# tangjiapeng/NSDP

Hardware: AMD Instinct MI355X
Metric: query-points/sec fwd+bwd (2048 surf pts, 8192 queries) (higher is better)
Workload: dtype f32; 1 GPU; forward.yaml TDNet train step (fwd + l2 loss + bwd + Adam), 32 shapes/GPU, 2048 surface + 8192 query points per shape, fp32 (dense layers as bf16x3 split products), procedural random-init weights; global_batch=32, n_surf=2048, n_query=8192, parallelism=dp1

## Files before the change

include/nsdp_hip.h:

```cpp
#ifndef NSDP_HIP_H_
#define NSDP_HIP_H_

#include <stddef.h>
#include <stdint.h>

#ifdef __cplusplus
extern "C" {
#endif

#define NSDP_EINVAL (-1)
#define NSDP_ENOSUP (-2)

int nsdp_abi_version(void);
const char *nsdp_last_error(void);
void nsdp_debug_set(int key, int value);
int nsdp_device_count(void);


int nsdp_furthest_point_sampling(const float *xyz, int B, int N, int nsamples, float *tmp,
                                 int32_t *idx_out, void *stream);

int nsdp_gather_points(const float *points, const int32_t *idx, int B, int C, int N, int M,
                       float *out, void *stream);
int nsdp_gather_points_grad(const float *grad_out, const int32_t *idx, int B, int C, int N, int M,
                            float *grad_points, void *stream);

int nsdp_group_points(const float *points, const int32_t *idx, int B, int C, int N, int NP, int NS,
                      float *out, void *stream);
int nsdp_group_points_grad(const float *grad_out, const int32_t *idx, int B, int C, int N, int NP,
                           int NS, float *grad_points, void *stream);

int nsdp_scatter_cm_lists_supported(int B, int C, int N, int E);
int nsdp_scatter_cm_lists(const float *grad_out, const int32_t *offsets, const int32_t *entries, int B, int C, int N,
                          int E, float *grad_points, void *stream);

int nsdp_three_interpolate_grad_lists_supported(int B, int c, int n, int m);
int nsdp_three_interpolate_grad_lists(const float *grad_out, const float *weight, const int32_t *offsets,
                                      const int32_t *entries, int B, int c, int n, int m, float *grad_points, void *stream);


int nsdp_ball_query(const float *new_xyz, const float *xyz, int B, int N, int M, float radius,
                    int nsample, int32_t *idx_out, void *stream);

int nsdp_three_nn(const float *unknown, const float *known, int B, int n, int m, float *dist2,
                  int32_t *idx, void *stream);
int nsdp_three_interpolate(const float *points, const int32_t *idx, const float *weight, int B,
                           int c, int m, int n, float *out, void *stream);
int nsdp_three_interpolate_grad(const float *grad_out, const int32_t *idx, const float *weight,
                                int B, int c, int n, int m, float *grad_points, void *stream);


int nsdp_knn(const float *query, const float *source, int B, int n, int m, int k, int32_t *idx_out,
             float *dist2_out, void *stream);

int nsdp_knn_ragged(const float *query, const int32_t *offsets, const float *source, int B, int cap, int m, int k,
                    int32_t *idx_out, float *dist2_out, void *stream);

int nsdp_gather_rows(const float *points, const int32_t *idx, int B, int N, int C, int S, float *out,
                     void *stream);
int nsdp_rel_coords4(const float *query, const float *source, const int32_t *idx, int B, int n, int m, int k, float sign,
                     float *out4, void *stream);
int nsdp_scatter_add_rows(const float *grad_out, const int32_t *idx, int B, int N, int C, int S,
                          float *grad_points, void *stream);


int nsdp_linear_f32(const float *X, const float *W, const float *bias, const float *residual,
                    const float *mask, const float *out_mask, float *Y, long long M, int N, int K,
                    int relu_in, int relu_out, void *stream);

long long nsdp_packed_weight_floats(int N, int K);
int nsdp_pack_weight_f32(const float *W, int N, int K, float *Wp, float *WpT, void *stream);

int nsdp_linear_wp_f32(const float *X, const float *Wp, const float *bias, const float *residual,
                       const float *mask, const float *out_mask, float *Y, long long M, int N, int K,
                       int relu_in, int relu_out, void *stream);

typedef struct {
  const float *W;
  void *Wp;
  void *WpT;
  int N, K;
  int kind;
  int reserved;
} NsdpPackDesc;
int nsdp_pack_weights_batched(const NsdpPackDesc *descs, int count, void *stream);

typedef struct {
  float *param;
  const float *grad;
  float *exp_avg;
  float *exp_avg_sq;
  float *step;
  long long numel;
} NsdpAdamDesc;
int nsdp_adam_chunk_elems(void);
int nsdp_adam_multi_f32(const NsdpAdamDesc *descs_dev, const int32_t *chunks_dev, int n_chunks, int32_t *done_dev,
                        const float *lr_dev, double lr, double beta1, double beta2, double eps, double weight_decay,
                        int maximize, void *stream);

long long nsdp_packed_weight_bf16x3_bytes(int N, int K, int transposed);
int nsdp_pack_weight_bf16x3(const float *W, int N, int K, void *Wp, void *WpT, void *stream);
int nsdp_linear_bf16x3_f32(const float *X, const void *Wp, const float *bias, const float *residual,
                           const float *mask, const float *out_mask, float *Y, long long M, int N, int K,
                           int relu_in, int relu_out, void *stream);

int nsdp_linear_bf16x3_gather_f32(const float *X, const void *Wp, const float *bias, const float *gq, int g_div, const float *gk,
                                  const int32_t *gidx, int g_rows_per_shape, int g_nsrc, float *Y, long long M, int N, int K,
                                  int relu_in, int relu_out, void *stream);

int nsdp_linear_bf16x3_signed_f32(const float *X, const void *Wp, const float *bias, const float *residual, float residual_sign,
                                  float *Y, long long M, int N, int K, int relu_in, int relu_out, void *stream);

int nsdp_linear_bf16x3_addend_f32(const float *X, const void *Wp, const float *bias, const float *residual, const float *mask,
                                  const float *out_mask, const float *addend, float *Y, long long M, int N, int K,
                                  int relu_out, void *stream);

int nsdp_linear_bf16x3_h0_supported(long long M, int N, int K);
int nsdp_linear_bf16x3_h0_f32(const float *X4, const float *W0, const float *b0, const void *Wp, const float *bias,
                              const float *gq, int g_div, const float *gk, const int32_t *gidx, int g_rows_per_shape, int g_nsrc,
                              float *Y, long long M, int N, int K, void *stream);

int nsdp_linear_bf16x3_k4tail_ok(long long M, int N, int K);
size_t nsdp_linear_bf16x3_k4tail_workspace_bytes(long long M, int N);
int nsdp_linear_bf16x3_k4tail_f32(const float *dY, const void *WpT, const float *X4, const float *W0, const float *b0,
                                  float *dW0, float *db0, long long M, int N, int K, int k_out, int accumulate, float *ws,
                                  size_t ws_bytes, void *stream);


size_t nsdp_linear_wgrad_workspace_bytes(long long M, int N, int K);
int nsdp_linear_wgrad_f32(const float *dY, const float *X, const float *mask, int relu_x, float *dW,
                          float *db, long long M, int N, int K, int accumulate, float *workspace,
                          size_t workspace_bytes, void *stream);
int nsdp_linear_wgrad_k4_remask_f32(const float *dY, const float *X, const float *W, const float *bias, float *dW,
                                    float *db, long long M, int N, int accumulate, float *workspace,
                                    size_t workspace_bytes, void *stream);

int nsdp_linear_wgrad_bf16x3_supported(long long M, int N, int K);
size_t nsdp_linear_wgrad_bf16x3_workspace_bytes(long long M, int N, int K);
int nsdp_linear_wgrad_bf16x3_f32(const float *dY, const float *X, const float *mask, int relu_x, float *dW,
                                 float *db, long long M, int N, int K, int accumulate, float *workspace,
                                 size_t workspace_bytes, void *stream);

typedef struct {
  const float *ws;
  float *dW, *db;
  int S, nta, ktb;
  int N, K;
  int accumulate;
  int reserved;
} NsdpWgradReduceDesc;
int nsdp_linear_wgrad_bf16x3_partials_f32(const float *dY, const float *X, const float *mask, int relu_x, float *dW,
                                          float *db, long long M, int N, int K, int accumulate, float *workspace,
                                          size_t workspace_bytes, NsdpWgradReduceDesc *desc_out, void *stream);
int nsdp_wgrad_bf16x3_reduce_batched(const NsdpWgradReduceDesc *descs, int count, void *stream);

int nsdp_attn_pre_fwd_bf16(const void *q, const void *kf, const void *pos, const int32_t *idx, int B, int n, int N, int k,
                           int d, int q_per_shape, void *u, void *stream);
int nsdp_attn_pre_bwd_bf16(const void *du, const int32_t *idx, int B, int n, int N, int k, int d, int q_per_shape,
                           float *dq, float *dkf, void *dpos_acc, void *stream);
int nsdp_attn_post_fwd_bf16(const void *a, const void *vf, const void *pos, const int32_t *idx, const void *a_g,
                            const void *v_g, const void *residual, int B, int n, int N, int k, int d, void *y, float *lse,
                            void *stream);
int nsdp_attn_post_bwd_bf16(const void *dy, const void *a, const void *vf, const void *pos, const int32_t *idx,
                            const void *a_g, const void *v_g, const void *y, const void *residual, const float *lse, int B,
                            int n, int N, int k, int d, void *da, void *dpos, float *dvf, float *da_g, float *dv_g,
                            void *stream);

long long nsdp_packed_weight_bf16_bytes(int N, int K, int transposed);
int nsdp_pack_weights_bf16(const NsdpPackDesc *descs, int count, void *stream);
int nsdp_linear_bf16(const void *X, const void *Wp, const float *bias, const void *residual, const void *mask,
                     const void *out_mask, void *Y, long long M, int N, int K, int relu_in, int relu_out, int out_f32,
                     void *stream);
size_t nsdp_linear_wgrad_bf16_workspace_bytes(long long M, int N, int K);
int nsdp_linear_wgrad_bf16_takes_mask(long long M, int N, int K);
int nsdp_linear_wgrad_bf16(const void *dY, const void *X, const void *mask, int relu_x, float *dW, float *db,
                           long long M, int N, int K, int accumulate, float *workspace, size_t workspace_bytes,
                           void *stream);

int nsdp_linear_wgrad_bf16x3_h0_supported(long long M, int N, int K);
int nsdp_linear_wgrad_bf16x3_h0_f32(const float *dY, const float *X4, const float *W0, const float *b0, float *dW, float *db,
                                    long long M, int N, int K, int accumulate, float *workspace, size_t workspace_bytes,
                                    NsdpWgradReduceDesc *desc_out, void *stream);

int nsdp_layout_g16_f32(const float *src, float *dst, long long M, int C, int to_g16, void *stream);
int nsdp_linear_bf16x3_g16_supported(long long M, int N, int K, int layout, int has_mask, int relu_in);
int nsdp_linear_bf16x3_g16_f32(const float *X, const void *Wp, const float *bias, const float *residual, const float *mask,
                               const float *out_mask, const float *addend, float *Y, long long M, int N, int K, int relu_in,
                               int relu_out, int layout, const unsigned char *mask_bits, unsigned char *bits_out, void *stream);
size_t nsdp_relu_bits_bytes(long long M, int C);
int nsdp_linear_wgrad_bf16x3_g16_supported(long long M, int N, int K, int layout, int has_mask);
int nsdp_linear_wgrad_bf16x3_g16_f32(const float *dY, const float *X, const float *mask, int relu_x, float *dW, float *db,
                                     long long M, int N, int K, int accumulate, float *workspace, size_t workspace_bytes,
                                     NsdpWgradReduceDesc *desc_out, int layout, const unsigned char *mask_bits, void *stream);

typedef struct {
  const float *ws;
  float *dW, *db;
  int S, N, K;
  int accumulate;
  int reserved;
} NsdpWgradB16ReduceDesc;
int nsdp_linear_wgrad_bf16_partials(const void *dY, const void *X, const void *mask, int relu_x, float *dW, float *db,
                                    long long M, int N, int K, int accumulate, float *workspace, size_t workspace_bytes,
                                    NsdpWgradB16ReduceDesc *desc_out, void *stream);
int nsdp_wgrad_bf16_reduce_batched(const NsdpWgradB16ReduceDesc *descs, int count, void *stream);
int nsdp_linear_wgrad_partials_f32(const float *dY, const float *X, const float *mask, int relu_x, float *dW, float *db,
                                   long long M, int N, int K, int accumulate, float *workspace, size_t workspace_bytes,
                                   NsdpWgradB16ReduceDesc *desc_out, void *stream);

int nsdp_bn_stats_bf16(const void *x, const void *addend, long long R, int C, float eps, float momentum,
                       float *running_mean, float *running_var, float *mean, float *invstd, float *workspace,
                       long long *num_batches_tracked, void *stream);
int nsdp_bn_train_fwd_bf16(const void *x, const void *addend, long long R, int C, float eps, float momentum, int updates,
                           float *running_mean, float *running_var, long long *num_batches_tracked, const float *gamma,
                           const float *beta, int relu, void *y, float *mean, float *invstd, float *workspace,
                           void *stream);
int nsdp_bn_apply_bf16(const void *x, const void *addend, const float *mean, const float *invstd, const float *gamma,
                       const float *beta, long long R, int C, int relu, void *y, void *stream);
int nsdp_bn_backward_bf16(const void *dy, const void *y_relu, const void *x, const void *addend, const float *mean,
                          const float *invstd, const float *gamma, long long R, int C, int training, void *dx,
                          float *dgamma, float *dbeta, float *workspace, void *stream);

int nsdp_knn_invert(const int32_t *idx, int B, int E, int N, int32_t *offsets, int32_t *entries, void *stream);
int nsdp_segment_sum_rows(const float *src, const int32_t *offsets, const int32_t *entries, int B, int E, int N, int d,
                          float scale, float *out, void *stream);
int nsdp_segment_sum_rows_bf16(const void *src, const int32_t *offsets, const int32_t *entries, int B, int E, int N, int d,
                               float scale, float *out, void *stream);
int nsdp_segment_sum_rows_add(const float *src, const int32_t *offsets, const int32_t *entries, int B, int E, int N, int d,
                              float scale, const float *addend, float *out, void *stream);
int nsdp_segment_sum_rows_add_bf16(const void *src, const int32_t *offsets, const int32_t *entries, int B, int E, int N, int d,
                                   float scale, const float *addend, float *out, void *stream);

size_t nsdp_scatter_rows_onehot_bf16_workspace_bytes(int B, long long rows, int N, int d);
int nsdp_scatter_rows_onehot_bf16(const void *src, const int32_t *idx, int B, long long rows, int N, int d, float *table,
                                  float *workspace, size_t workspace_bytes, void *stream);
size_t nsdp_scatter_rows_onehot_f32_workspace_bytes(int B, long long rows, int N, int d);
int nsdp_scatter_rows_onehot_f32(const float *src, const int32_t *idx, int B, long long rows, int N, int d, float *table,
                                 float *workspace, size_t workspace_bytes, void *stream);

int nsdp_linear_k4_bf16(const float *X, const float *W, const float *bias, void *Y, long long M, int N, int relu_out,
                        void *stream);
size_t nsdp_linear_wgrad_k4_bf16_workspace_bytes(long long M, int N);
int nsdp_linear_wgrad_k4_bf16(const void *dY, const float *X, const void *mask, float *dW, float *db, long long M, int N,
                              float *workspace, size_t workspace_bytes, void *stream);


int nsdp_attn_pre_fwd(const float *q, const float *kf, const float *pos, const int32_t *idx, int B, int n,
                      int N, int k, int d, int q_per_shape, float *u, void *stream);
int nsdp_attn_pre_bwd(const float *du, const int32_t *idx, int B, int n, int N, int k, int d,
                      int q_per_shape, float *dq, float *dkf, float *dpos_acc, void *stream);
int nsdp_attn_pre_bwd_sub(const float *du, const int32_t *idx, int B, int n, int N, int k, int d, const float *dq_sub, float *dq,
                          void *stream);
int nsdp_attn_pre_bwd_sub_bf16(const void *du, const int32_t *idx, int B, int n, int N, int k, int d, const void *dq_sub, float *dq,
                               void *stream);
int nsdp_attn_post_fwd(const float *a, const float *vf, const float *pos, const int32_t *idx,
                       const float *a_g, const float *v_g, const float *residual, int B, int n, int N,
                       int k, int d, float *y, float *lse, void *stream);
int nsdp_attn_post_bwd(const float *dy, const float *a, const float *vf, const float *pos,
                       const int32_t *idx, const float *a_g, const float *v_g, const float *y,
                       const float *residual, const float *lse, int B, int n, int N, int k, int d,
                       float *da, float *dpos, float *dvf, float *da_g, float *dv_g, void *stream);

int nsdp_attn_post_fwd_q(const float *a, const float *vk, const float *u, const int32_t *idx, const float *qsub,
                         const float *residual, int B, int n, int N, int k, int d, float *y, float *lse, void *stream);
int nsdp_attn_post_bwd_q(const float *dy, const float *a, const float *vk, const float *u, const int32_t *idx, const float *qsub,
                         const float *y, const float *residual, const float *lse, int B, int n, int N, int k, int d,
                         float *da, float *dpos, float *dvf, void *stream);

size_t nsdp_attn_post_bwd_det_workspace_bytes(int B, int n, int k, int d);
int nsdp_attn_post_bwd_det(const float *dy, const float *a, const float *vf, const float *pos, const int32_t *idx,
                           const float *a_g, const float *v_g, const float *y, const float *residual, const float *lse,
                           int B, int n, int N, int k, int d, float *da, float *dpos, float *da_g, float *dv_g,
                           float *workspace, size_t workspace_bytes, void *stream);
int nsdp_attn_post_bwd_det_bf16(const void *dy, const void *a, const void *vf, const void *pos, const int32_t *idx,
                                const void *a_g, const void *v_g, const void *y, const void *residual, const float *lse,
                                int B, int n, int N, int k, int d, void *da, void *dpos, float *da_g, float *dv_g,
                                float *workspace, size_t workspace_bytes, void *stream);


int nsdp_decoder_fused_fwd(const float *xyz_q, const float *anchors, const int32_t *idx, const float *qk,
                           const float *vtab, const float *a_g, const float *v_g,
                           const float *const *weights, int n_weights, int B, int NQ, int A, int KN, int D,
                           int H, float *out, void *stream);

int nsdp_decoder_fused_fwd_bf16(const float *xyz_q, const float *anchors, const int32_t *idx, const float *qk,
                                const float *vtab, const float *a_g, const float *v_g,
                                const void *const *weights, int n_weights, int B, int NQ, int A, int KN, int D,
                                int H, float *out, void *stream);

int nsdp_decoder_fused_fwd_ragged(const float *xyz_q, const int32_t *offsets, const float *anchors, const int32_t *idx,
                                  const float *qk, const float *vtab, const float *a_g, const float *v_g,
                                  const float *const *weights, int n_weights, int B, int cap, int A, int KN, int D,
                                  int H, float *out, void *stream);
int nsdp_decoder_fused_fwd_bf16_ragged(const float *xyz_q, const int32_t *offsets, const float *anchors, const int32_t *idx,
                                       const float *qk, const float *vtab, const float *a_g, const float *v_g,
                                       const void *const *weights, int n_weights, int B, int cap, int A, int KN, int D,
                                       int H, float *out, void *stream);

size_t nsdp_bn_workspace_bytes(int C);
int nsdp_bn_stats(const float *x, const float *addend, long long R, int C, float eps, float momentum,
                  float *running_mean, float *running_var, float *mean, float *invstd, float *workspace,
                  long long *num_batches_tracked, void *stream);
int nsdp_bn_train_fwd(const float *x, const float *addend, long long R, int C, float eps, float momentum, int updates,
                      float *running_mean, float *running_var, long long *num_batches_tracked, const float *gamma,
                      const float *beta, int relu, float *y, float *mean, float *invstd, float *workspace, void *stream);
int nsdp_bn_apply(const float *x, const float *addend, const float *mean, const float *invstd,
                  const float *gamma, const float *beta, long long R, int C, int relu, float *y, void *stream);
int nsdp_bn_backward(const float *dy, const float *y_relu, const float *x, const float *addend,
                     const float *mean, const float *invstd, const float *gamma, long long R, int C,
                     int training, float *dx, float *dgamma, float *dbeta, float *workspace, void *stream);

void nsdp_prof_enable(int on);
void nsdp_prof_enable_kinds(unsigned mask);
int nsdp_prof_num_kinds(void);
void nsdp_trace_enable(int on);
int nsdp_trace_read(char *buf, int capacity);
const char *nsdp_prof_name(int kind);
int nsdp_prof_collect(int kind, long long *launches, double *total_ms, double *flops, double *bytes);

int nsdp_graph_exec_create(void *graph, int max_streams, void **out_handle);
int nsdp_graph_exec_info(void *handle, int *nodes, int *kernels, int *streams, int *cross_edges, int *own_graph_nodes);
int nsdp_graph_exec_launch(void *handle, void *stream);
int nsdp_graph_exec_launch_timed(void *handle, void *stream, const char *name_substr, long long *launches, double *total_ms);
int nsdp_graph_exec_destroy(void *handle);

#ifdef __cplusplus
}
#endif
#endif
```

nsdp_amd/build.py:

```python
from __future__ import annotations

import os
import subprocess
import sys
from concurrent.futures import ThreadPoolExecutor

HERE = os.path.dirname(os.path.abspath(__file__))
CSRC = os.path.join(HERE, "csrc")
LIBDIR = os.path.join(HERE, "lib")
OBJDIR = os.path.join(LIBDIR, "obj")
SO = os.path.join(LIBDIR, "libnsdp_hip.so")
HEADER = os.path.join(os.path.dirname(HERE), "include", "nsdp_hip.h")

HIPCC = os.environ.get("HIPCC", "/opt/rocm/bin/hipcc")
COMMON = ["--offload-arch=gfx950", "-O3", "-std=c++17", "-fPIC", "-Wall", "-Wno-unused-function",
          "-munsafe-fp-atomics"]
EXACT = ["-ffp-contract=off"]
FAST = ["-ffp-contract=fast"]
PER_FILE = {
    "fps.hip": EXACT,
    "knn.hip": EXACT,
    "pointnet2_ops.hip": EXACT,
    "adam.hip": EXACT,
    "wgrad_bf16x3.hip": FAST + ["-O2", "-fno-slp-vectorize"],
    "gemm_bf16x3.hip": FAST + ["-fno-slp-vectorize"],
    "gemm_bf16x3_g16.hip": FAST + ["-fno-slp-vectorize"],
}


def sources():
    return sorted(f for f in os.listdir(CSRC) if f.endswith(".hip"))


def _deps_mtime():
    hs = [os.path.join(CSRC, f) for f in os.listdir(CSRC) if f.endswith(".h")] + [HEADER, os.path.abspath(__file__)]
    return max(os.path.getmtime(h) for h in hs)


def _compile(src, force):
    obj = os.path.join(OBJDIR, src[:-4] + ".o")
    path = os.path.join(CSRC, src)
    if (not force and os.path.exists(obj)
            and os.path.getmtime(obj) >= max(os.path.getmtime(path), _deps_mtime())):
        return obj, False
    cmd = [HIPCC] + COMMON + PER_FILE.get(src, FAST) + ["-c", path, "-o", obj]
    subprocess.check_call(cmd)
    return obj, True


def build(force: bool = False, verbose: bool = False) -> str:
    os.makedirs(OBJDIR, exist_ok=True)
    with ThreadPoolExecutor(max_workers=min(8, os.cpu_count() or 1)) as ex:
        results = list(ex.map(lambda s: _compile(s, force), sources()))
    objs = [o for o, _ in results]
    if force or any(c for _, c in results) or not os.path.exists(SO):
        subprocess.check_call([HIPCC, "--offload-arch=gfx950", "-shared", "-fPIC", "-o", SO] + objs)
        if verbose:
            print("linked", SO)
    return SO


if __name__ == "__main__":
    print(build(force="--force" in sys.argv, verbose=True))
```

nsdp_amd/csrc/x3_kernel.h:

```cpp
#pragma once
#include <stdlib.h>

#include <type_traits>

#include "common.h"
#include "k4.h"
#include "pack_bodies.h"
#include "prof.h"

namespace nsdp {
extern int g_x3_dbg;
extern thread_local int g_x3_side_reserve;
}

namespace {

using f32x4 = __attribute__((ext_vector_type(4))) float;
using f32x2 = __attribute__((ext_vector_type(2))) float;
using u32x4 = __attribute__((ext_vector_type(4))) unsigned;
using bf16x2 = __attribute__((ext_vector_type(2))) __bf16;
using bf16x8 = __attribute__((ext_vector_type(8))) __bf16;

typedef __attribute__((address_space(3))) void *lds_ptr_t;
typedef const __attribute__((address_space(1))) void *gbl_ptr_t;

using nsdp::g_x3_dbg;
using nsdp::g_x3_side_reserve;

#ifdef NSDP_X3_TIMING
__device__ unsigned long long g_x3_timers[8];
#define X3_T(var) const unsigned long long var = __builtin_readcyclecounter()
#define X3_ADD(i, a, b) t_acc[i] += (b) - (a)
#else
#define X3_T(var)
#define X3_ADD(i, a, b)
#endif

struct X3Params {
  const float *X;
  const void *Wp;
  const float *bias, *residual, *mask, *out_mask;
  float *Y;
  long long M;
  int N, K;
  int relu_in, relu_out;
  int dbg;
  const float *gq, *gk;
  const int32_t *gidx;
  int g_div, g_rps, g_nsrc;
  float res_sign = 1.f;
  const float *addend = nullptr;
  const float *t_x4 = nullptr, *t_w0 = nullptr, *t_b0 = nullptr;
  float *t_ws = nullptr;
  const float *h_x4 = nullptr, *h_w0 = nullptr, *h_b0 = nullptr;
  const unsigned char *bits = nullptr;
  unsigned char *bits_out = nullptr;
};

constexpr int kLayX = 1;
constexpr int kLayY = 2;
constexpr int kLayR = 4;

__device__ __forceinline__ void split_pair(float x0, float x1, unsigned &h, unsigned &m, unsigned &l) {
  h = __builtin_bit_cast(unsigned, __builtin_convertvector(f32x2{x0, x1}, bf16x2));
  const float r0 = x0 - __builtin_bit_cast(float, h << 16), r1 = x1 - __builtin_bit_cast(float, h & 0xffff0000u);
  m = __builtin_bit_cast(unsigned, __builtin_convertvector(f32x2{r0, r1}, bf16x2));
  const float s0 = r0 - __builtin_bit_cast(float, m << 16), s1 = r1 - __builtin_bit_cast(float, m & 0xffff0000u);
  l = __builtin_bit_cast(unsigned, __builtin_convertvector(f32x2{s0, s1}, bf16x2));
}

__device__ __forceinline__ f32x4 mfma_bf16(u32x4 a, u32x4 b, f32x4 c) {
  return __builtin_amdgcn_mfma_f32_16x16x32_bf16(__builtin_bit_cast(bf16x8, a), __builtin_bit_cast(bf16x8, b), c, 0, 0, 0);
}

template <int I, int N, typename F>
__device__ __forceinline__ void static_for(F &&f) {
  if constexpr (I < N) {
    f(std::integral_constant<int, I>{});
    static_for<I + 1, N>(f);
  }
}

#define NSDP_DPP4(CTRL, A, B, C, D)                                                                                              \
  asm("s_nop 1\n\t"                                                                                                              \
      "v_add_f32_dpp %0, %0, %0 " CTRL "\n\tv_add_f32_dpp %1, %1, %1 " CTRL "\n\tv_add_f32_dpp %2, %2, %2 " CTRL "\n\t"            \
      "v_add_f32_dpp %3, %3, %3 " CTRL "\n\ts_nop 1"                                                                              \
      : "+v"(A), "+v"(B), "+v"(C), "+v"(D))
#define NSDP_DPP16(CTRL, T)                                                                                                      \
  asm("s_nop 1\n\t"                                                                                                              \
      "v_add_f32_dpp %0, %0, %0 " CTRL "\n\tv_add_f32_dpp %1, %1, %1 " CTRL "\n\tv_add_f32_dpp %2, %2, %2 " CTRL "\n\t"            \
      "v_add_f32_dpp %3, %3, %3 " CTRL "\n\tv_add_f32_dpp %4, %4, %4 " CTRL "\n\tv_add_f32_dpp %5, %5, %5 " CTRL "\n\t"            \
      "v_add_f32_dpp %6, %6, %6 " CTRL "\n\tv_add_f32_dpp %7, %7, %7 " CTRL "\n\tv_add_f32_dpp %8, %8, %8 " CTRL "\n\t"            \
      "v_add_f32_dpp %9, %9, %9 " CTRL "\n\tv_add_f32_dpp %10, %10, %10 " CTRL "\n\tv_add_f32_dpp %11, %11, %11 " CTRL "\n\t"      \
      "v_add_f32_dpp %12, %12, %12 " CTRL "\n\tv_add_f32_dpp %13, %13, %13 " CTRL "\n\tv_add_f32_dpp %14, %14, %14 " CTRL "\n\t"   \
      "v_add_f32_dpp %15, %15, %15 " CTRL "\n\ts_nop 1"                                                                           \
      : "+v"(T[0]), "+v"(T[1]), "+v"(T[2]), "+v"(T[3]), "+v"(T[4]), "+v"(T[5]), "+v"(T[6]), "+v"(T[7]), "+v"(T[8]), "+v"(T[9]),   \
        "+v"(T[10]), "+v"(T[11]), "+v"(T[12]), "+v"(T[13]), "+v"(T[14]), "+v"(T[15]))
template <bool K3>
__device__ __forceinline__ void row16_sum20(float (&t)[20]) {
  if constexpr (K3) {
    float u[16] = {t[0], t[1], t[2], t[4], t[5], t[6], t[8], t[9], t[10], t[12], t[13], t[14], t[16], t[17], t[18], t[19]};
    NSDP_DPP16("quad_perm:[1,0,3,2] row_mask:0xf bank_mask:0xf", u);
    NSDP_DPP16("quad_perm:[2,3,0,1] row_mask:0xf bank_mask:0xf", u);
    NSDP_DPP16("row_half_mirror row_mask:0xf bank_mask:0xf", u);
    NSDP_DPP16("row_mirror row_mask:0xf bank_mask:0xf", u);
    t[0] = u[0]; t[1] = u[1]; t[2] = u[2]; t[4] = u[3]; t[5] = u[4]; t[6] = u[5]; t[8] = u[6]; t[9] = u[7]; t[10] = u[8];
    t[12] = u[9]; t[13] = u[10]; t[14] = u[11]; t[16] = u[12]; t[17] = u[13]; t[18] = u[14]; t[19] = u[15];
  } else {
    NSDP_DPP16("quad_perm:[1,0,3,2] row_mask:0xf bank_mask:0xf", t);
    NSDP_DPP4("quad_perm:[1,0,3,2] row_mask:0xf bank_mask:0xf", t[16], t[17], t[18], t[19]);
    NSDP_DPP16("quad_perm:[2,3,0,1] row_mask:0xf bank_mask:0xf", t);
    NSDP_DPP4("quad_perm:[2,3,0,1] row_mask:0xf bank_mask:0xf", t[16], t[17], t[18], t[19]);
    NSDP_DPP16("row_half_mirror row_mask:0xf bank_mask:0xf", t);
    NSDP_DPP4("row_half_mirror row_mask:0xf bank_mask:0xf", t[16], t[17], t[18], t[19]);
    NSDP_DPP16("row_mirror row_mask:0xf bank_mask:0xf", t);
    NSDP_DPP4("row_mirror row_mask:0xf bank_mask:0xf", t[16], t[17], t[18], t[19]);
  }
}
#undef NSDP_DPP16
#undef NSDP_DPP4

__device__ __forceinline__ void xload(f32x4 &dst, const float *lane_ptr) {
  asm volatile("global_load_dwordx4 %0, %1, off" : "=v"(dst) : "v"(lane_ptr));
}
__device__ __forceinline__ void bload(unsigned &dst, const unsigned char *lane_ptr) {
  asm volatile("global_load_ubyte %0, %1, off" : "=v"(dst) : "v"(lane_ptr));
}


template <int OFF>
__device__ __forceinline__ void lds_read(u32x4 &dst, unsigned lane_addr) {
  asm volatile("ds_read_b128 %0, %1 offset:%2" : "=v"(dst) : "v"(lane_addr), "n"(OFF));
}
__device__ __forceinline__ void lds_wait(u32x4 &a, u32x4 &b, u32x4 &c) {
  asm volatile("s_waitcnt lgkmcnt(0)" : "+v"(a), "+v"(b), "+v"(c));
}

typedef __attribute__((address_space(3))) f32x4 *lds_f4_ptr;
template <int OFF>
__device__ __forceinline__ void lds_read_f4(f32x4 &dst, unsigned addr) {
  dst = *reinterpret_cast<lds_f4_ptr>(static_cast<uintptr_t>(addr + static_cast<unsigned>(OFF)));
}
template <int OFF>
__device__ __forceinline__ void lds_write_f4(unsigned addr, f32x4 v) {
  *reinterpret_cast<lds_f4_ptr>(static_cast<uintptr_t>(addr + static_cast<unsigned>(OFF))) = v;
}
template <int CNT>
__device__ __forceinline__ void lgkm_wait(f32x4 &) {}
__device__ __forceinline__ void store_f4(unsigned byte_off, f32x4 v, float *uniform_base) {
  *reinterpret_cast<f32x4 *>(reinterpret_cast<char *>(uniform_base) + byte_off) = v;
}

template <int MT, int NT, int PRE, int WV, bool XREG = false, int KBM = 2, int GATHER = 0, int TAIL = 0, int LAY = 0>
__global__ __launch_bounds__(WV * 64, XREG ? 2 : 1) void linear_bf16x3_kernel(X3Params p) {
  constexpr bool kXG = (LAY & kLayX) != 0, kYG = (LAY & kLayY) != 0, kRG = (LAY & kLayR) != 0;
  static_assert(!kYG || (!GATHER && !TAIL), "G16 output: plain epilogue forms");
  static_assert(!kXG || PRE != 3, "G16 input: there is no X in the H0 forms");
  static_assert(PRE != 4 || kXG, "ReLU bits belong to G16 operands");
  constexpr bool kMasked = PRE == 1 || PRE == 4;
  static_assert(!GATHER || PRE == 0 || PRE == 3, "the gathered addend belongs to the plain-prologue forms");
  static_assert(!TAIL || (PRE == 0 && !GATHER), "the K = 4 tail belongs to the plain-prologue forms");
  constexpr bool WRES = KBM > 2;
  constexpr bool kH0 = PRE == 3;
  constexpr bool kXLds = !kMasked && !XREG && !kH0;
  constexpr int kWTile = NT * 3 * 64;
  constexpr int kXTile = kXLds ? 2 * WV * MT * 2 * 64 : 1;
  constexpr bool kTwoPerCu = XREG || (NT <= 8 && WV == 4);
  constexpr int kCap = (kTwoPerCu ? 80 : 160) * 64;
  constexpr int kBiasLds = NT * 4;
  constexpr int kH0Rows = kH0 ? ((NT * 16 + 31) / 32) * 32 : 0;
  constexpr int kH0XRows = kH0 ? 2 * WV * MT * 16 : 0;
  constexpr int kH0Lds = kH0Rows + kH0Rows / 4 + kH0XRows;
  constexpr int kExtFree = kCap - KBM * kWTile - kXTile - kBiasLds - kH0Lds;
  constexpr bool kStage = !WRES && kExtFree >= 0 && !TAIL && !kYG;
  constexpr int kExtWant = WV * NT * 64 - kWTile;
  constexpr int kExt = !kStage ? 0 : (kExtWant < 0 ? 0 : (kExtFree < 0 ? 0 : (kExtWant < kExtFree ? kExtWant : kExtFree)));
  constexpr int kPerWave = (kWTile + kExt) / WV;
  constexpr int kTppFit = kPerWave / 64 < NT ? kPerWave / 64 : NT;
  constexpr int kTppCap = (NT == 13 && (WV == 8 || XREG)) ? 5 : 8;
  constexpr int kTppMax = kTppFit < kTppCap ? kTppFit : kTppCap;
  constexpr int kPasses = kStage ? (NT + kTppMax - 1) / kTppMax : 1;
  constexpr int kTpp = (NT + kPasses - 1) / kPasses;
  static_assert(!kStage || kTppMax >= 1, "epilogue staging: no room for a 16 x 16 tile per wave");
  __shared__ __attribute__((aligned(16))) u32x4 wlds[KBM * kWTile + kExt];
  __shared__ __attribute__((aligned(16))) u32x4 xbuf[kXLds ? 2 : 1][kXLds ? WV : 1][kXLds ? MT * 2 * 64 : 1];
  __shared__ __attribute__((aligned(16))) float bias_lds[(kStage || TAIL) ? NT * 16 : 4];
  __shared__ __attribute__((aligned(16))) f32x4 t_w0lds[TAIL ? NT * 16 : 1];
  __shared__ __attribute__((aligned(16))) f32x4 t_x4lds[TAIL ? WV * 64 : 1];
  __shared__ __attribute__((aligned(16))) f32x4 h_w0lds[kH0 ? kH0Rows : 1];
  __shared__ __attribute__((aligned(16))) float h_b0lds[kH0 ? kH0Rows : 4];
  __shared__ __attribute__((aligned(16))) f32x4 h_x4lds[kH0 ? 2 : 1][kH0 ? WV : 1][kH0 ? MT * 16 : 1];
  static_assert(!TAIL || !WRES, "the K = 4 tail needs 1 KiB of LDS per wave and 272 B per n tile next to the weight buffers");
  static_assert(!TAIL || MT * 16 <= 64, "the K = 4 tail stages one input row per lane");
  auto wbuf_at = [&](int b) -> u32x4 * { return wlds + b * kWTile + (b >= 1 ? kExt : 0); };
  const int lane = threadIdx.x & 63;
  const int wave = __builtin_amdgcn_readfirstlane(threadIdx.x >> 6);
  const int li = lane & 15, g = lane >> 4;
  const int K = p.K, N = p.N;
  const int KB = (K + 31) >> 5;
  const int ntiles = (N + 15) >> 4;
  constexpr long long kRowsWg = static_cast<long long>(WV) * MT * 16;
  const long long wg_tiles = (p.M + kRowsWg - 1) / kRowsWg;
  const long long stride = gridDim.x;
  long long tile = blockIdx.x;

  const float *xa[MT], *xn[MT];
  const float *ma[MT], *mn[MT];
  auto set_rows = [&](long long t, const float **x, const float **m) {
#pragma unroll
    for (int mt = 0; mt < MT; ++mt) {
      long long r = (t * WV + wave) * (MT * 16) + mt * 16 + li;
      r = r < p.M ? r : (p.M - 1);
      const long long ro = kXG ? (r & ~15LL) * K + (r & 15) * 4 : r * K;
      x[mt] = p.X + ro;
      m[mt] = PRE == 1 ? p.mask + ro : nullptr;
      if constexpr (PRE == 4)
        m[mt] = reinterpret_cast<const float *>(p.bits + (r >> 4) * (static_cast<long long>((K + 31) >> 5) * 64) + (r & 15) * 4 + g);
    }
  };
  set_rows(tile, xa, ma);
  set_rows(tile + stride, xn, mn);
  f32x4 h_xs[kH0 ? MT : 1];
  int h_kb = 0;
  unsigned h_par = 0;
  auto h_rows = [&](long long t, unsigned buf) {
    if (lane < MT * 16) {
      long long r = (t * WV + wave) * (MT * 16) + lane;
      r = r < p.M ? r : (p.M - 1);
      __builtin_amdgcn_global_load_lds((gbl_ptr_t)(p.h_x4 + r * 4), (lds_ptr_t)(&h_x4lds[buf][wave][0]), 16, 0, 0);
    }
  };
  auto h_take = [&](unsigned buf) {
#pragma unroll
    for (int mt = 0; mt < MT; ++mt) h_xs[mt] = h_x4lds[buf][wave][mt * 16 + li];
  };
  if constexpr (kH0) {
    h_rows(tile, 0u);
    h_rows(tile + stride, 1u);
    asm volatile("s_waitcnt vmcnt(0)" ::: "memory");
    h_take(0u);
  }

  const char *wlane = static_cast<const char *>(p.Wp) + lane * 16;
  auto stage = [&](int kb, int buf) {
    const int pieces = ntiles * 3;
    for (int q = wave; q < pieces; q += WV)
      __builtin_amdgcn_global_load_lds((gbl_ptr_t)(wlane + ((static_cast<long long>(kb) * pieces + q) << 10)),
                                       (lds_ptr_t)(wbuf_at(buf) + q * 64), 16, 0, 0);
  };
  const unsigned lds0 = static_cast<unsigned>(reinterpret_cast<uintptr_t>((lds_ptr_t)(&wlds[lane])));
  const unsigned ldsw = static_cast<unsigned>(reinterpret_cast<uintptr_t>((lds_ptr_t)(&wlds[0])));
  const unsigned ldsb = static_cast<unsigned>(reinterpret_cast<uintptr_t>((lds_ptr_t)(&bias_lds[0])));
  constexpr unsigned kBufBytes = NT * 3 * 1024;
  constexpr unsigned kExtBytes = kExt * 16;

  f32x4 raw[kXLds ? 1 : MT][2], rawm[kXLds ? 1 : MT][2];
  unsigned rawb[PRE == 4 ? MT : 1];
  auto xissue = [&](const float *const *x, const float *const *m, int kb, unsigned xb) {
    if constexpr (kH0) return;
#pragma unroll
    for (int mt = 0; mt < MT; ++mt)
#pragma unroll
      for (int hf = 0; hf < 2; ++hf) {
        int ko = kb * 32 + 16 * hf + 4 * g;
        ko = ko < K ? ko : (K - 4);
        if constexpr (kXG) ko *= 16;
        if constexpr (kXLds) {
          const float *src = x[mt] + ko;
          if (p.dbg & 1024) src = x[0] - li * K + (((kb * MT * 2 + mt * 2 + hf) * 256) % 6144) + lane * 4;
          __builtin_amdgcn_global_load_lds((gbl_ptr_t)src, (lds_ptr_t)(&xbuf[xb][wave][(mt * 2 + hf) * 64]), 16, 0, 0);
        } else {
          xload(raw[mt][hf], x[mt] + ko);
          if constexpr (PRE == 1) xload(rawm[mt][hf], m[mt] + ko);
          if constexpr (PRE == 4) {
            if (hf == 0) bload(rawb[mt], reinterpret_cast<const unsigned char *>(m[mt]) + kb * 64);
          }
        }
      }
  };
  auto xwait = [&]() {
    if constexpr (kXLds || kH0) {
      asm volatile("s_waitcnt vmcnt(0)" ::: "memory");
    } else {
#pragma unroll
      for (int mt = 0; mt < MT; ++mt) {
        asm volatile("s_waitcnt vmcnt(0)" : "+v"(raw[mt][0]), "+v"(raw[mt][1]));
        if constexpr (PRE == 1) asm volatile("s_waitcnt vmcnt(0)" : "+v"(rawm[mt][0]), "+v"(rawm[mt][1]));
        if constexpr (PRE == 4) asm volatile("s_waitcnt vmcnt(0)" : "+v"(rawb[mt]));
      }
    }
  };
  struct Planes {
    u32x4 h[MT], m[MT], l[MT];
  };
  auto convert_pair = [&](Planes &pl, int mt, int pr, unsigned xb) {
    if constexpr (kH0) {
      const int k0 = h_kb * 32 + 16 * (pr >> 1) + 4 * g + 2 * (pr & 1);
      const f32x4 wa = h_w0lds[k0], wb = h_w0lds[k0 + 1];
      const f32x2 bb = *reinterpret_cast<const f32x2 *>(&h_b0lds[k0]);
      const float4 xq = make_float4(h_xs[mt][0], h_xs[mt][1], h_xs[mt][2], h_xs[mt][3]);
      const f32x2 pre = nsdp::k4_preact_pair(xq, f32x2{wa[0], wa[1]}, f32x2{wa[2], wa[3]}, f32x2{wb[0], wb[1]}, f32x2{wb[2], wb[3]}, bb);
      unsigned h, m, l;
      split_pair(fmaxf(pre[0], 0.f), fmaxf(pre[1], 0.f), h, m, l);
      pl.h[mt][pr] = h; pl.m[mt][pr] = m; pl.l[mt][pr] = l;
      return;
    }
    f32x4 v;
    if constexpr (kXLds) {
      v = __builtin_bit_cast(f32x4, xbuf[xb][wave][(mt * 2 + (pr >> 1)) * 64 + lane]);
    } else {
      v = raw[mt][pr >> 1];
      if constexpr (PRE == 1) {
        const f32x4 mk = rawm[mt][pr >> 1];
#pragma unroll
        for (int c = 0; c < 4; ++c) v[c] = mk[c] > 0.f ? v[c] : 0.f;
      }
      if constexpr (PRE == 4) {
        const unsigned nib = rawb[mt] >> (4 * (pr >> 1));
#pragma unroll
        for (int c = 0; c < 4; ++c) v[c] = ((nib >> c) & 1u) ? v[c] : 0.f;
      }
    }
    if (PRE == 2) {
#pragma unroll
      for (int c = 0; c < 4; ++c) v[c] = __builtin_amdgcn_fmed3f(v[c], 0.f, __builtin_inff());
    }
    unsigned h, m, l;
    split_pair(v[2 * (pr & 1)], v[2 * (pr & 1) + 1], h, m, l);
    pl.h[mt][pr] = h; pl.m[mt][pr] = m; pl.l[mt][pr] = l;
  };

  auto pair_mt = [](int i) { return kH0 ? i % MT : i >> 2; };
  auto pair_pr = [](int i) { return kH0 ? i / MT : i & 3; };
  Planes cur, nxt;
  if constexpr (kH0) {
    for (int c = threadIdx.x; c < kH0Rows; c += WV * 64) h_b0lds[c] = (p.h_b0 && c < K) ? p.h_b0[c] : 0.f;
    for (int j = threadIdx.x; j < kH0Rows / 2; j += WV * 64) nsdp::k4_pair_table(p.h_w0, K, j, h_w0lds[2 * j], h_w0lds[2 * j + 1]);
    __syncthreads();
  }
  if constexpr (kStage) {
    for (int c = threadIdx.x; c < NT * 16; c += WV * 64) bias_lds[c] = (p.bias && c < p.N) ? p.bias[c] : 0.f;
  }
  if constexpr (TAIL) {
    for (int c = threadIdx.x; c < NT * 16; c += WV * 64) {
      bias_lds[c] = (p.t_b0 && c < p.N) ? p.t_b0[c] : 0.f;
      t_w0lds[c] = c < p.N ? *reinterpret_cast<const f32x4 *>(p.t_w0 + static_cast<long long>(c) * 4) : f32x4{0.f, 0.f, 0.f, 0.f};
    }
  }
  if (wg_tiles >= 4 * stride) {
    int phase = static_cast<int>(blockIdx.x & 7);
    if (WV == 4 && gridDim.x > 256 && blockIdx.x >= gridDim.x / 2) phase = (phase + 4) & 7;
    for (int i = 0; i < phase * KB; ++i) __builtin_amdgcn_s_sleep(10);
  }
  if constexpr (WRES) {
    for (int kb = 0; kb < KB; ++kb) stage(kb, kb);
  } else {
    stage(0, 0);
  }
  xissue(xa, ma, 0, 0u);
  if constexpr (kXLds) xissue(xa, ma, 1, 1u);
  xwait();
#pragma unroll
  for (int mt = 0; mt < MT; ++mt)
#pragma unroll
    for (int pr = 0; pr < 4; ++pr) convert_pair(cur, mt, pr, 0u);
  if constexpr (!kXLds) {
    xissue(xa, ma, 1, 0u);
    xwait();
  }
  __syncthreads();

  constexpr int kConvSteps = NT > 4 ? 4 : NT - 1;
  constexpr int kConvFirst = kXLds ? NT - kConvSteps : 0;
  constexpr int kPairs = MT * 4;
  constexpr int kPerStep = (kPairs + kConvSteps - 1) / kConvSteps;
  constexpr int kValuPerMfma = (kPerStep * ((PRE == 1 || PRE == 4) ? 13 : PRE == 2 ? 10 : PRE == 3 ? 21 : 9) + 6 * MT - 1) / (6 * MT);

#ifdef NSDP_X3_TIMING
  unsigned long long t_acc[8] = {0, 0, 0, 0, 0, 0, 0, 0};
  const unsigned long long t_begin = __builtin_readcyclecounter();
#endif
  unsigned gs = 0;
  for (;;) {
    X3_T(t_tile0);
    const long long row0 = (tile * WV + wave) * (MT * 16);
    const bool next_tile = tile + stride < wg_tiles;
    if constexpr (TAIL) {
      long long r = row0 + (lane < MT * 16 ? lane : MT * 16 - 1);
      r = r < p.M ? r : p.M - 1;
      __builtin_amdgcn_global_load_lds((gbl_ptr_t)(p.t_x4 + r * 4), (lds_ptr_t)(&t_x4lds[wave * 64]), 16, 0, 0);
    }
    int li_t = li, g_t = g;
    asm volatile("" : "+v"(li_t), "+v"(g_t));
    f32x4 acc[MT][NT];
    unsigned gqo[GATHER == 1 ? MT : 1], gko[GATHER ? MT : 1];
    if constexpr (GATHER) {
#pragma unroll
      for (int mt = 0; mt < MT; ++mt) {
        long long row = row0 + mt * 16 + li_t;
        row = row < p.M ? row : (p.M - 1);
        const unsigned r32 = static_cast<unsigned>(row);
        if constexpr (GATHER == 1) gqo[mt] = (r32 / static_cast<unsigned>(p.g_div)) * static_cast<unsigned>(N);
        gko[mt] = ((r32 / static_cast<unsigned>(p.g_rps)) * static_cast<unsigned>(p.g_nsrc) + static_cast<unsigned>(p.gidx[row])) *
                  static_cast<unsigned>(N);
      }
    }
    if (!GATHER && p.residual) {
#pragma unroll
      for (int mt = 0; mt < MT; ++mt) {
        long long row = row0 + mt * 16 + li_t;
        row = row < p.M ? row : (p.M - 1);
#pragma unroll
        for (int nt = 0; nt < NT; ++nt) {
          int col = nt * 16 + 4 * g_t;
          col = col + 4 <= N ? col : (N - 4);
          const long long ro = kRG ? (row & ~15LL) * N + (row & 15) * 4 + col * 16 : row * N + col;
          const float4 v = *reinterpret_cast<const float4 *>(p.residual + ro);
          acc[mt][nt] = f32x4{v.x, v.y, v.z, v.w};
          if constexpr (PRE == 0) acc[mt][nt] *= p.res_sign;
        }
      }
    } else {
#pragma unroll
      for (int mt = 0; mt < MT; ++mt)
#pragma unroll
        for (int nt = 0; nt < NT; ++nt) acc[mt][nt] = f32x4{0.f, 0.f, 0.f, 0.f};
    }

    X3_T(t_tile1);
    X3_ADD(4, t_tile0, t_tile1);
    for (int kb = 0; kb < KB; ++kb, ++gs) {
      X3_T(t_k0);
      const unsigned buf = gs & 1u;
      const bool more = kb + 1 < KB || next_tile;
      if constexpr (!WRES) {
        if (more && !(p.dbg & 1)) stage(kb + 1 < KB ? kb + 1 : 0, buf ^ 1u);
      }
      bool x_issued = false;
      if constexpr (kXLds) {
        if (kb + 2 < KB) { xissue(xa, ma, kb + 2, buf); x_issued = true; }
        else if (next_tile) { xissue(xn, mn, kb + 2 - KB, buf); x_issued = true; }
      }
      auto xwait_older = [&]() {
        if (x_issued) asm volatile("s_waitcnt vmcnt(%0)" ::"n"(MT * 2) : "memory");
        else asm volatile("s_waitcnt vmcnt(0)" ::: "memory");
      };
      if constexpr (kH0) {
        const bool wrap = kb + 1 >= KB;
        h_kb = wrap ? 0 : kb + 1;
        if (wrap) h_take(h_par ^ 1u);
      }
      const unsigned wsel = WRES ? static_cast<unsigned>(kb) : buf;
      const unsigned wl_addr = lds0 + wsel * kBufBytes + (wsel >= 1u ? kExtBytes : 0u);
      u32x4 wh, wm, wl;
      lds_read<0>(wh, wl_addr); lds_read<1024>(wm, wl_addr); lds_read<2048>(wl, wl_addr);
      lds_wait(wh, wm, wl);
      static_for<0, NT>([&](auto I) {
        constexpr int nt = decltype(I)::value;
        u32x4 nh, nm, nl;
        if constexpr (nt + 1 < NT) {
          lds_read<(nt + 1) * 3072>(nh, wl_addr);
          if (!(p.dbg & 512)) {
            lds_read<(nt + 1) * 3072 + 1024>(nm, wl_addr);
            lds_read<(nt + 1) * 3072 + 2048>(nl, wl_addr);
          } else {
            nm = nh; nl = nh;
          }
        }
        if constexpr (!kXLds && !kH0 && nt == kConvFirst + kConvSteps) {
          if (kb + 2 < KB) xissue(xa, ma, kb + 2, 0u);
          else if (next_tile) xissue(xn, mn, kb + 2 - KB, 0u);
        }
        if constexpr (kXLds && nt == kConvFirst) xwait_older();
        if constexpr (nt >= kConvFirst && nt < kConvFirst + kConvSteps) {
#pragma unroll
          for (int i = 0; i < kPerStep; ++i) {
            constexpr int base = (nt - kConvFirst) * kPerStep;
            if (base + i < kPairs) convert_pair(nxt, pair_mt(base + i), pair_pr(base + i), buf ^ 1u);
          }
        }
#pragma unroll
        for (int mt = 0; mt < MT; ++mt) acc[mt][nt] = mfma_bf16(wh, cur.l[mt], acc[mt][nt]);
#pragma unroll
        for (int mt = 0; mt < MT; ++mt) acc[mt][nt] = mfma_bf16(wl, cur.h[mt], acc[mt][nt]);
#pragma unroll
        for (int mt = 0; mt < MT; ++mt) acc[mt][nt] = mfma_bf16(wm, cur.m[mt], acc[mt][nt]);
#pragma unroll
        for (int mt = 0; mt < MT; ++mt) acc[mt][nt] = mfma_bf16(wh, cur.m[mt], acc[mt][nt]);
#pragma unroll
        for (int mt = 0; mt < MT; ++mt) acc[mt][nt] = mfma_bf16(wm, cur.h[mt], acc[mt][nt]);
#pragma unroll
        for (int mt = 0; mt < MT; ++mt) acc[mt][nt] = mfma_bf16(wh, cur.h[mt], acc[mt][nt]);
        if constexpr (nt >= kConvFirst && nt < kConvFirst + kConvSteps) {
#pragma unroll
          for (int i = 0; i < 6 * MT; ++i) {
            __builtin_amdgcn_sched_group_barrier(0x008, 1, 0);
            __builtin_amdgcn_sched_group_barrier(0x002, kValuPerMfma, 0);
          }
        }
#pragma unroll
        for (int mt = 0; mt < MT; ++mt) asm volatile("" : "+a"(acc[mt][nt]));
        if constexpr (nt >= kConvFirst && nt < kConvFirst + kConvSteps) {
#pragma unroll
          for (int i = 0; i < kPerStep; ++i) {
            constexpr int base = (nt - kConvFirst) * kPerStep;
            if (base + i < kPairs) {
              const int mt = pair_mt(base + i), pr = pair_pr(base + i);
              asm volatile("" : "+v"(nxt.h[mt][pr]), "+v"(nxt.m[mt][pr]), "+v"(nxt.l[mt][pr]));
            }
          }
        }
        if constexpr (nt + 1 < NT) {
          lds_wait(nh, nm, nl);
          wh = nh; wm = nm; wl = nl;
        }
      });
      X3_T(t_k1);
      if constexpr (kXLds) xwait_older();
      else xwait();
      X3_T(t_k2);
      if constexpr (!WRES) {
        asm volatile("s_waitcnt lgkmcnt(0)" ::: "memory");
        __builtin_amdgcn_s_barrier();
      }
      asm volatile("" ::: "memory");
      X3_T(t_k3);
      X3_ADD(0, t_k0, t_k1); X3_ADD(1, t_k1, t_k2); X3_ADD(2, t_k2, t_k3);
      cur = nxt;
    }

    X3_T(t_e0);
    if (row0 < p.M && !(p.dbg & 8)) {
      const bool full_rows = row0 + MT * 16 <= p.M;
      int li_e = li, g_e = g;
      asm volatile("" : "+v"(li_e), "+v"(g_e));
      float4 bias4[NT];
#pragma unroll
      for (int nt = 0; nt < NT; ++nt) bias4[nt] = make_float4(0.f, 0.f, 0.f, 0.f);
      if (p.bias && (!kStage || (p.dbg & (8192 | 16384 | 32768)))) {
#pragma unroll
        for (int nt = 0; nt < NT; ++nt) {
          const int col = nt * 16 + 4 * g_e;
          bias4[nt] = *reinterpret_cast<const float4 *>(p.bias + (col + 4 <= N ? col : (N - 4)));
        }
      }
      auto gload = [&](int nt, f32x4 *ga, f32x4 *gb) {
        if constexpr (GATHER) {
          int col = nt * 16 + 4 * g_e;
          col = col + 4 <= N ? col : (N - 4);
#pragma unroll
          for (int mt = 0; mt < MT; ++mt) {
            if constexpr (GATHER == 1) ga[mt] = *reinterpret_cast<const f32x4 *>(p.gq + gqo[mt] + col);
            gb[mt] = *reinterpret_cast<const f32x4 *>(p.gk + gko[mt] + col);
          }
        }
      };
      auto otile = [&](int nt, auto has_omask, auto guarded, const f32x4 *ga = nullptr, const f32x4 *gb = nullptr) {
        const int col = nt * 16 + 4 * g_e;
        const bool cv = col + 4 <= N;
        const int colc = cv ? col : (N - 4);
        const float4 bv = bias4[nt];
#pragma unroll
        for (int mt = 0; mt < MT; ++mt) {
          const long long row = row0 + mt * 16 + li_e;
          const bool rv = !decltype(guarded)::value || row < p.M;
          const long long rowc = rv ? row : (p.M - 1);
          float4 v = make_float4(acc[mt][nt][0] + bv.x, acc[mt][nt][1] + bv.y, acc[mt][nt][2] + bv.z, acc[mt][nt][3] + bv.w);
          if constexpr (GATHER) {
            const f32x4 d = GATHER == 2 ? gb[mt] : ga[mt] - gb[mt];
            v.x += d[0]; v.y += d[1]; v.z += d[2]; v.w += d[3];
          }
          if (p.relu_out) { v.x = fmaxf(v.x, 0.f); v.y = fmaxf(v.y, 0.f); v.z = fmaxf(v.z, 0.f); v.w = fmaxf(v.w, 0.f); }
          if (decltype(has_omask)::value) {
            const float4 om = *reinterpret_cast<const float4 *>(p.out_mask + rowc * N + colc);
            v.x = om.x > 0.f ? v.x : 0.f; v.y = om.y > 0.f ? v.y : 0.f; v.z = om.z > 0.f ? v.z : 0.f; v.w = om.w > 0.f ? v.w : 0.f;
          }
          if constexpr (decltype(has_omask)::value == 2) {
            const float4 ad = *reinterpret_cast<const float4 *>(p.addend + rowc * N + colc);
            v.x += ad.x; v.y += ad.y; v.z += ad.z; v.w += ad.w;
          }
          const f32x4 vv = {v.x, v.y, v.z, v.w};
          if (decltype(guarded)::value) {
            if (cv && rv) {
              if (p.dbg & 64) __builtin_nontemporal_store(vv, reinterpret_cast<f32x4 *>(p.Y + rowc * N + colc));
              else *reinterpret_cast<f32x4 *>(p.Y + rowc * N + colc) = vv;
            }
          } else {
            if (p.dbg & 64) __builtin_nontemporal_store(vv, reinterpret_cast<f32x4 *>(p.Y + row * N + col));
            else if (p.dbg & 2048)
              *reinterpret_cast<f32x4 *>(p.Y + row0 * N + (((mt * NT + nt) * 256) % 6144) + (li_e + 16 * g_e) * 4) = vv;
            else *reinterpret_cast<f32x4 *>(p.Y + row * N + col) = vv;
          }
        }
      };
      auto staged = [&](auto has_omask) {
        const unsigned buf_last = (gs - 1u) & 1u;
        const unsigned ebase = ldsw + (buf_last ? kBufBytes : 0u) + static_cast<unsigned>(wave) * (kPerWave * 16u);
        const unsigned lane_e = static_cast<unsigned>(li_e + 16 * g_e);
        const unsigned rd = ebase + lane_e * 16u;
        float *ytile = p.Y + row0 * N;
        const float *mtile = decltype(has_omask)::value ? p.out_mask + row0 * N : nullptr;
        const float *atile = decltype(has_omask)::value == 2 ? p.addend + row0 * N : nullptr;
        const int rows_left = p.M - row0 < MT * 16 ? static_cast<int>(p.M - row0) : MT * 16;
        static_for<0, MT>([&](auto MI) {
          constexpr int mt = decltype(MI)::value;
          static_for<0, kPasses>([&](auto PI) {
            constexpr int pass = decltype(PI)::value;
            constexpr int nt0 = pass * kTpp;
            constexpr int ntn = (NT - nt0) < kTpp ? (NT - nt0) : kTpp;
            constexpr unsigned pitch = ntn * 64u;
            const unsigned wr = ebase + static_cast<unsigned>(li_e) * pitch + static_cast<unsigned>(g_e) * 16u;
            const int valid = (N - nt0 * 16) * 4 < static_cast<int>(pitch) ? (N - nt0 * 16) * 4 : static_cast<int>(pitch);
            unsigned off[ntn];
            bool live[ntn];
            f32x4 om[decltype(has_omask)::value ? ntn : 1];
            f32x4 ad[decltype(has_omask)::value == 2 ? ntn : 1];
            f32x4 gka[GATHER == 2 ? ntn : 1];
            static_for<0, ntn>([&](auto CI) {
              constexpr int i = decltype(CI)::value;
              const unsigned f = static_cast<unsigned>(i) * 1024u + lane_e * 16u;
              const unsigned r = f / pitch, cb = f - r * pitch;
              off[i] = ((static_cast<unsigned>(mt) * 16u + r) * static_cast<unsigned>(N) + static_cast<unsigned>(nt0) * 16u) * 4u + cb;
              live[i] = static_cast<int>(cb) < valid && static_cast<int>(mt * 16 + r) < rows_left;
              if constexpr (decltype(has_omask)::value) {
                om[i] = live[i] ? *reinterpret_cast<const f32x4 *>(reinterpret_cast<const char *>(mtile) + off[i]) : f32x4{0.f, 0.f, 0.f, 0.f};
              }
              if constexpr (decltype(has_omask)::value == 2) {
                ad[i] = live[i] ? *reinterpret_cast<const f32x4 *>(reinterpret_cast<const char *>(atile) + off[i]) : f32x4{0.f, 0.f, 0.f, 0.f};
              }
              if constexpr (GATHER == 2) {
                const unsigned cbytes = static_cast<unsigned>(nt0) * 64u + cb;
                const unsigned ko = static_cast<unsigned>(__builtin_amdgcn_ds_bpermute(static_cast<int>(r * 4u), static_cast<int>(gko[mt])));
                gka[i] = live[i] ? *reinterpret_cast<const f32x4 *>(reinterpret_cast<const char *>(p.gk + ko) + cbytes) : f32x4{0.f, 0.f, 0.f, 0.f};
              }
            });
            f32x4 gav[GATHER == 1 ? ntn : 1], gbv[GATHER == 1 ? ntn : 1];
            if constexpr (GATHER == 1) {
              static_for<0, ntn>([&](auto TI) {
                constexpr int t = decltype(TI)::value;
                int col = (nt0 + t) * 16 + 4 * g_e;
                col = col + 4 <= N ? col : (N - 4);
                gav[t] = *reinterpret_cast<const f32x4 *>(p.gq + gqo[mt] + col);
                gbv[t] = *reinterpret_cast<const f32x4 *>(p.gk + gko[mt] + col);
              });
            }
            f32x4 bvv[ntn];
            static_for<0, ntn>([&](auto TI) {
              constexpr int t = decltype(TI)::value;
              lds_read_f4<(nt0 + t) * 64>(bvv[t], ldsb + static_cast<unsigned>(16 * g_e));
            });
            static_for<0, ntn>([&](auto TI) {
              constexpr int t = decltype(TI)::value;
              constexpr int nt = nt0 + t;
              lgkm_wait<ntn - 1 - t>(bvv[t]);
              f32x4 v = acc[mt][nt] + bvv[t];
              if constexpr (GATHER == 1) v += gav[t] - gbv[t];
              if (p.relu_out) {
#pragma unroll
                for (int c = 0; c < 4; ++c) v[c] = fmaxf(v[c], 0.f);
              }
              lds_write_f4<t * 64>(wr, v);
            });
            asm volatile("s_waitcnt lgkmcnt(0)" ::: "memory");
            f32x4 back[ntn];
            static_for<0, ntn>([&](auto CI) {
              constexpr int i = decltype(CI)::value;
              lds_read_f4<i * 1024>(back[i], rd);
            });
            static_for<0, ntn>([&](auto CI) {
              constexpr int i = decltype(CI)::value;
              lgkm_wait<ntn - 1 - i>(back[i]);
              f32x4 v = back[i];
              if constexpr (decltype(has_omask)::value) {
#pragma unroll
                for (int c = 0; c < 4; ++c) v[c] = om[i][c] > 0.f ? v[c] : 0.f;
              }
              if constexpr (decltype(has_omask)::value == 2) v += ad[i];
              if constexpr (GATHER == 2) v += gka[i];
              if (live[i]) store_f4(off[i], v, ytile);
            });
          });
        });
      };
      auto direct_tail = [&]() __attribute__((always_inline)) {
        f32x4 xr[MT];
        bool rvm[MT];
        const unsigned x4a = static_cast<unsigned>(reinterpret_cast<uintptr_t>((lds_ptr_t)(&t_x4lds[wave * 64]))) + static_cast<unsigned>(li_e) * 16u;
        const unsigned w0a = static_cast<unsigned>(reinterpret_cast<uintptr_t>((lds_ptr_t)(&t_w0lds[0]))) + static_cast<unsigned>(g_e) * 64u;
        static_for<0, MT>([&](auto MI) {
          constexpr int mt = decltype(MI)::value;
          rvm[mt] = row0 + mt * 16 + li_e < p.M;
          lds_read_f4<mt * 256>(xr[mt], x4a);
        });
        float *wsp = p.t_ws + (tile * WV + wave) * static_cast<long long>(NT * 80) + g_e * 20;
        static_for<0, NT>([&](auto NI) {
          constexpr int nt = decltype(NI)::value;
          const int col = nt * 16 + 4 * g_e;
          const bool cv = col < N;
          f32x4 w0[4], b0;
          static_for<0, 4>([&](auto CI) {
            constexpr int c = decltype(CI)::value;
            lds_read_f4<(nt * 16 + c) * 16>(w0[c], w0a);
          });
          lds_read_f4<nt * 64>(b0, ldsb + static_cast<unsigned>(16 * g_e));
          float ta[20];
#pragma unroll
          for (int v = 0; v < 20; ++v) ta[v] = 0.f;
#pragma unroll
          for (int mt = 0; mt < MT; ++mt) {
            const float4 xq = make_float4(xr[mt][0], xr[mt][1], xr[mt][2], xr[mt][3]);
            const bool ok = rvm[mt] && cv;
#pragma unroll
            for (int c = 0; c < 4; ++c) {
              const float pre = nsdp::k4_preact_n(xq, make_float4(w0[c][0], w0[c][1], w0[c][2], w0[c][3]), b0[c], c);
              const float d = (ok && pre > 0.f) ? acc[mt][nt][c] : 0.f;
              ta[16 + c] += d;
#pragma unroll
              for (int k = 0; k < (TAIL == 2 ? 3 : 4); ++k) ta[4 * c + k] += d * xr[mt][k];
            }
          }
          row16_sum20<TAIL == 2>(ta);
          if (li_e == 0) {
#pragma unroll
            for (int j = 0; j < 5; ++j)
              *reinterpret_cast<f32x4 *>(wsp + nt * 80 + j * 4) = f32x4{ta[4 * j], ta[4 * j + 1], ta[4 * j + 2], ta[4 * j + 3]};
          }
        });
      };
      auto g16_out = [&]() __attribute__((always_inline)) {
        float *ytile = p.Y + row0 * N + (li_e + 16 * g_e) * 4;
        unsigned char *btile = p.bits_out ? p.bits_out + (row0 >> 4) * (static_cast<long long>((N + 31) >> 5) * 64) + li_e * 4 + g_e : nullptr;
        static_for<0, MT>([&](auto MI) __attribute__((always_inline)) {
          constexpr int mt = decltype(MI)::value;
          if (row0 + mt * 16 < p.M) {
            unsigned byte = 0;
            static_for<0, NT>([&](auto NI) __attribute__((always_inline)) {
              constexpr int nt = decltype(NI)::value;
              const float4 bv = bias4[nt];
              f32x4 v = {acc[mt][nt][0] + bv.x, acc[mt][nt][1] + bv.y, acc[mt][nt][2] + bv.z, acc[mt][nt][3] + bv.w};
              if (p.relu_out) {
#pragma unroll
                for (int c = 0; c < 4; ++c) v[c] = fmaxf(v[c], 0.f);
              }
              const bool cv = nt * 16 + 4 * g_e + 4 <= N;
              if (cv) *reinterpret_cast<f32x4 *>(ytile + mt * 16 * N + nt * 256) = v;
              if (btile) {
                const unsigned nib = cv ? ((v[0] > 0.f ? 1u : 0u) | (v[1] > 0.f ? 2u : 0u) | (v[2] > 0.f ? 4u : 0u) | (v[3] > 0.f ? 8u : 0u)) : 0u;
                byte = (nt & 1) ? (byte | (nib << 4)) : nib;
                if ((nt & 1) || nt == NT - 1) {
                  if (nt * 16 < ((N + 31) >> 5) * 32) btile[mt * (((N + 31) >> 5) * 64) + (nt >> 1) * 64] = static_cast<unsigned char>(byte);
                }
              }
            });
          }
        });
      };
      auto epilogue = [&](auto has_omask) {
        const int full_tiles = N >> 4;
        if constexpr (TAIL) {
          direct_tail();
          return;
        }
        if constexpr (kYG) {
          g16_out();
          return;
        }
        if constexpr (kStage) {
          staged(has_omask);
          return;
        }
        if constexpr (GATHER) {
          f32x4 ga[2][MT], gb[2][MT];
          gload(0, ga[0], gb[0]);
          static_for<0, NT>([&](auto I) {
            constexpr int nt = decltype(I)::value;
            if (nt * 16 < N) {
              if constexpr (nt + 1 < NT) {
                if ((nt + 1) * 16 < N) gload(nt + 1, ga[(nt + 1) & 1], gb[(nt + 1) & 1]);
              }
              otile(nt, has_omask, std::true_type{}, ga[nt & 1], gb[nt & 1]);
            }
          });
          return;
        }
        if (full_rows) {
#pragma unroll
          for (int nt = 0; nt < NT; ++nt) {
            if (nt < full_tiles) otile(nt, has_omask, std::false_type{});
            else if (nt * 16 < N) otile(nt, has_omask, std::true_type{});
          }
        } else {
#pragma unroll
          for (int nt = 0; nt < NT; ++nt)
            if (nt * 16 < N) otile(nt, has_omask, std::true_type{});
        }
      };
      if (p.out_mask) {
        if constexpr (kMasked) {
          if (p.addend) epilogue(std::integral_constant<int, 2>{});
          else epilogue(std::true_type{});
        } else {
          epilogue(std::true_type{});
        }
      } else {
        epilogue(std::false_type{});
      }
    }

    X3_T(t_e1);
    X3_ADD(3, t_e0, t_e1);
    if (!next_tile) break;
    if constexpr (kStage) {
      asm volatile("s_waitcnt lgkmcnt(0)" ::: "memory");
      __builtin_amdgcn_s_barrier();
      asm volatile("" ::: "memory");
    }
    tile += stride;
#pragma unroll
    for (int mt = 0; mt < MT; ++mt) { xa[mt] = xn[mt]; ma[mt] = mn[mt]; }
    set_rows(tile + stride, xn, mn);
    if constexpr (kH0) {
      h_rows(tile + stride, h_par);
      h_par ^= 1u;
    }
  }
#ifdef NSDP_X3_TIMING
  t_acc[5] = __builtin_readcyclecounter() - t_begin;
  if (lane == 0)
    for (int i = 0; i < 6; ++i) atomicAdd(&g_x3_timers[i], t_acc[i]);
#endif
}

template <int MT, int NT, int PRE, int WV, bool XREG = false, int KBM = 2, int GATHER = 0, int LAY = 0>
void launch_x3_pre(const X3Params &p, hipStream_t st, int wgs_per_cu = 1) {
  const long long rows_per_wg = static_cast<long long>(WV) * MT * 16;
  const long long wg_tiles = (p.M + rows_per_wg - 1) / rows_per_wg;
  static const int reserve_env = getenv("NSDP_X3_RESERVE_CUS") ? atoi(getenv("NSDP_X3_RESERVE_CUS")) : 0;
  const int reserve = g_x3_side_reserve > 0 && g_x3_side_reserve < nsdp::num_cus() ? g_x3_side_reserve : reserve_env;
  const long long slots = static_cast<long long>(nsdp::num_cus() - reserve) * wgs_per_cu;
  const unsigned grid = static_cast<unsigned>(wg_tiles < slots ? wg_tiles : slots);
  NSDP_TRACE("linear_bf16x3<%d,%d,%d,%d,%d>x%d%s%s%s", MT, NT, PRE, WV, static_cast<int>(XREG), wgs_per_cu, KBM > 2 ? " wres" : "",
             GATHER == 2 ? " gather1" : GATHER ? " gather" : "",
             LAY == 0 ? "" : LAY == 1 ? " g16:x" : LAY == 2 ? " g16:y" : LAY == 3 ? " g16:xy" : LAY == 4 ? " g16:r" : LAY == 5 ? " g16:xr" : LAY == 6 ? " g16:yr" : " g16:xyr");
  hipLaunchKernelGGL((linear_bf16x3_kernel<MT, NT, PRE, WV, XREG, KBM, GATHER, 0, LAY>), dim3(grid), dim3(WV * 64), 0, st, p);
}

}
```

nsdp_amd/hip_linear.py:

```python
from __future__ import annotations

import ctypes
import os
import weakref

import torch
import torch.nn.functional as F

from . import precision
from ._lib import check, fptr, lib, on_device, optptr, stream_ptr

_ll = ctypes.c_longlong
_ci = ctypes.c_int


def _fwd(x2, w, b, residual, mask, out_mask, relu_in, relu_out):
    M, K = x2.shape
    N = w.shape[0]
    y = torch.empty((M, N), dtype=torch.float32, device=x2.device)
    with on_device(x2):
        check(lib().nsdp_linear_f32(fptr(x2, "x"), fptr(w, "weight"), optptr(b), optptr(residual), optptr(mask),
                                    optptr(out_mask), fptr(y), _ll(M), _ci(N), _ci(K), _ci(int(relu_in)),
                                    _ci(int(relu_out)), stream_ptr()), "nsdp_linear_f32")
    return y


def pack_weight(w, fwd=True, transposed=False):
    N, K = w.shape
    L = lib()
    L.nsdp_packed_weight_floats.restype = ctypes.c_longlong
    n = int(L.nsdp_packed_weight_floats(_ci(N), _ci(K)))
    wp = torch.empty(n, dtype=torch.float32, device=w.device) if fwd else None
    wpt = torch.empty(n, dtype=torch.float32, device=w.device) if transposed else None
    with on_device(w):
        check(L.nsdp_pack_weight_f32(fptr(w, "weight"), _ci(N), _ci(K), optptr(wp), optptr(wpt), stream_ptr()),
              "nsdp_pack_weight_f32")
    return wp, wpt


def _fwd_wp(x2, wp, N, b, residual, mask, out_mask, relu_in, relu_out):
    M, K = x2.shape
    y = torch.empty((M, N), dtype=torch.float32, device=x2.device)
    with on_device(x2):
        check(lib().nsdp_linear_wp_f32(fptr(x2, "x"), fptr(wp, "packed weight"), optptr(b), optptr(residual),
                                       optptr(mask), optptr(out_mask), fptr(y), _ll(M), _ci(N), _ci(K),
                                       _ci(int(relu_in)), _ci(int(relu_out)), stream_ptr()), "nsdp_linear_wp_f32")
    return y


def pack_weight_x3(w, fwd=True, transposed=False):
    N, K = w.shape
    L = lib()
    L.nsdp_packed_weight_bf16x3_bytes.restype = ctypes.c_longlong
    wp = wpt = None
    if fwd:
        wp = torch.empty(int(L.nsdp_packed_weight_bf16x3_bytes(_ci(N), _ci(K), _ci(0))), dtype=torch.uint8, device=w.device)
    if transposed:
        wpt = torch.empty(int(L.nsdp_packed_weight_bf16x3_bytes(_ci(N), _ci(K), _ci(1))), dtype=torch.uint8, device=w.device)
    with on_device(w):
        check(L.nsdp_pack_weight_bf16x3(fptr(w, "weight"), _ci(N), _ci(K), optptr(wp), optptr(wpt), stream_ptr()),
              "nsdp_pack_weight_bf16x3")
    return wp, wpt


def _fwd_x3(x2, wp, N, b, residual, mask, out_mask, relu_in, relu_out, res_sign=1.0, addend=None):
    M, K = x2.shape
    y = torch.empty((M, N), dtype=torch.float32, device=x2.device)
    if addend is not None:
        if mask is None or out_mask is None or relu_in or res_sign != 1.0:
            raise ValueError("a post-mask addend needs mask and out_mask, no input ReLU, an unsigned residual")
        with on_device(x2):
            check(lib().nsdp_linear_bf16x3_addend_f32(fptr(x2, "x"), ctypes.c_void_p(wp.data_ptr()), optptr(b), optptr(residual),
                                                      fptr(mask, "mask"), fptr(out_mask, "out_mask"), fptr(addend, "addend"),
                                                      fptr(y), _ll(M), _ci(N), _ci(K), _ci(int(relu_out)), stream_ptr()),
                  "nsdp_linear_bf16x3_addend_f32")
        return y
    if res_sign != 1.0:
        if residual is None or mask is not None or out_mask is not None:
            raise ValueError("a signed residual needs a residual and no masks")
        with on_device(x2):
            check(lib().nsdp_linear_bf16x3_signed_f32(fptr(x2, "x"), ctypes.c_void_p(wp.data_ptr()), optptr(b),
                                                      fptr(residual, "residual"), ctypes.c_float(res_sign), fptr(y), _ll(M),
                                                      _ci(N), _ci(K), _ci(int(relu_in)), _ci(int(relu_out)), stream_ptr()),
                  "nsdp_linear_bf16x3_signed_f32")
        return y
    with on_device(x2):
        check(lib().nsdp_linear_bf16x3_f32(fptr(x2, "x"), ctypes.c_void_p(wp.data_ptr()), optptr(b), optptr(residual),
                                           optptr(mask), optptr(out_mask), fptr(y), _ll(M), _ci(N), _ci(K),
                                           _ci(int(relu_in)), _ci(int(relu_out)), stream_ptr()),
              "nsdp_linear_bf16x3_f32")
    return y


def _fwd_x3_gather(x2, wp, N, b, gather, relu_in, relu_out):
    gq, g_div, gk, gidx, rps, nsrc = gather
    M, K = x2.shape
    if (gq is not None and gq.shape[-1] != N) or gk.shape[-1] != N or gidx.numel() != M:
        raise ValueError("init_gather: table width / index count do not match the layer")
    y = torch.empty((M, N), dtype=torch.float32, device=x2.device)
    with on_device(x2):
        check(lib().nsdp_linear_bf16x3_gather_f32(fptr(x2, "x"), ctypes.c_void_p(wp.data_ptr()), optptr(b), optptr(gq),
                                                  _ci(int(g_div)), fptr(gk, "gk"), ctypes.c_void_p(gidx.data_ptr()),
                                                  _ci(int(rps)), _ci(int(nsrc)), fptr(y), _ll(M), _ci(N), _ci(K),
                                                  _ci(int(relu_in)), _ci(int(relu_out)), stream_ptr()),
              "nsdp_linear_bf16x3_gather_f32")
    return y


G16 = os.environ.get("NSDP_G16", "1") != "0"
LAY_X, LAY_Y = 1, 2
G16_BITS = os.environ.get("NSDP_G16_BITS", "1") != "0"


def relu_bits(M, C, device):
    L = lib()
    L.nsdp_relu_bits_bytes.restype = ctypes.c_size_t
    return torch.empty(int(L.nsdp_relu_bits_bytes(_ll(M), _ci(C))), dtype=torch.uint8, device=device)


def _fwd_x3_g16(x2, wp, N, b, residual, mask, out_mask, relu_in, relu_out, layout, addend=None, mask_bits=None, bits_out=None):
    M, K = x2.shape
    y = torch.empty((M, N), dtype=torch.float32, device=x2.device)
    with on_device(x2):
        check(lib().nsdp_linear_bf16x3_g16_f32(fptr(x2, "x"), ctypes.c_void_p(wp.data_ptr()), optptr(b), optptr(residual),
                                               optptr(mask), optptr(out_mask), optptr(addend), fptr(y), _ll(M), _ci(N), _ci(K),
                                               _ci(int(relu_in)), _ci(int(relu_out)), _ci(int(layout)),
                                               ctypes.c_void_p(mask_bits.data_ptr() if mask_bits is not None else None),
                                               ctypes.c_void_p(bits_out.data_ptr() if bits_out is not None else None), stream_ptr()),
              "nsdp_linear_bf16x3_g16_f32")
    return y


def to_g16(t, back=False):
    t2 = t.reshape(-1, t.shape[-1]).contiguous()
    out = torch.empty_like(t2)
    with on_device(t2):
        check(lib().nsdp_layout_g16_f32(fptr(t2, "src"), fptr(out), _ll(t2.shape[0]), _ci(t2.shape[1]), _ci(0 if back else 1),
                                        stream_ptr()), "nsdp_layout_g16_f32")
    return out.reshape(t.shape)


def _wgrad_g16_fn(layout, bits=None):
    def fn(dy2, x2, mask, relu_x, want_db, out=None):
        if bits is not None:
            mask = None
        M, N = dy2.shape
        K = x2.shape[1]
        L = lib()
        L.nsdp_linear_wgrad_bf16x3_workspace_bytes.restype = ctypes.c_size_t
        nbytes = int(L.nsdp_linear_wgrad_bf16x3_workspace_bytes(_ll(M), _ci(N), _ci(K)))
        ws = torch.empty(max(nbytes // 4, 1), dtype=torch.float32, device=dy2.device)
        dw, db, acc = wgrad_out(out, N, K, want_db, dy2.device)
        batch = _cur_reduce if BATCH_REDUCE > 0 else None
        desc = _ReduceDesc() if batch is not None else None
        with on_device(dy2):
            if batch is not None:
                ptrs = {dw.data_ptr()} | ({db.data_ptr()} if db is not None else set())
                if ptrs & batch["targets"]:
                    _flush_reduce(batch)
            check(L.nsdp_linear_wgrad_bf16x3_g16_f32(fptr(dy2, "dy"), fptr(x2, "x"), optptr(mask), _ci(int(relu_x)), fptr(dw),
                                                     optptr(db), _ll(M), _ci(N), _ci(K), _ci(acc), fptr(ws), ctypes.c_size_t(nbytes),
                                                     ctypes.byref(desc) if desc is not None else None, _ci(int(layout)),
                                                     ctypes.c_void_p(bits.data_ptr() if bits is not None else None), stream_ptr()),
                  "nsdp_linear_wgrad_bf16x3_g16_f32")
            if batch is not None:
                batch["descs"].append(desc)
                batch["keep"].append((ws, dw, db, bits))
                batch["targets"] |= ptrs
                if len(batch["descs"]) + len(batch["descs_b16"]) >= BATCH_REDUCE:
                    _flush_reduce(batch)
        return dw, db
    fn.batched_reduce = True
    fn.extra_tensors = (bits,) if bits is not None else ()
    return fn


def g16_pair_ok(M, K, H, N, relu_in0=False, train=True):
    if not G16 or precision.is_bf16() or M % 16:
        return False
    L = lib()
    ok = (_x3_ok(M, H, K) and _x3_ok(M, N, H)
          and L.nsdp_linear_bf16x3_g16_supported(_ll(M), _ci(H), _ci(K), _ci(LAY_Y), _ci(0), _ci(int(relu_in0)))
          and L.nsdp_linear_bf16x3_g16_supported(_ll(M), _ci(N), _ci(H), _ci(LAY_X), _ci(0), _ci(0)))
    if not ok or not train:
        return bool(ok)
    return bool(_x3_ok(M, H, N) and _x3_ok(M, K, H) and M >= _X3_MIN_ROWS_WGRAD
                and L.nsdp_linear_bf16x3_g16_supported(_ll(M), _ci(H), _ci(N), _ci(LAY_Y), _ci(0), _ci(0))
                and L.nsdp_linear_bf16x3_g16_supported(_ll(M), _ci(K), _ci(H), _ci(LAY_X), _ci(1), _ci(0))
                and L.nsdp_linear_wgrad_bf16x3_g16_supported(_ll(M), _ci(N), _ci(H), _ci(2), _ci(0))
                and L.nsdp_linear_wgrad_bf16x3_g16_supported(_ll(M), _ci(H), _ci(K), _ci(1), _ci(1)))


def gather_init_ok(M, N, K):
    return _x3_ok(M, N, K) and M < 2 ** 31 and not precision.is_bf16()


def wgrad_out(out, N, K, want_db, device):
    if out is not None:
        dw, db = out
        if (tuple(dw.shape) == (N, K) and dw.dtype is torch.float32 and dw.is_contiguous()
                and (not want_db or (db is not None and db.dtype is torch.float32 and db.is_contiguous()))):
            return dw, (db if want_db else None), 1
    dw = torch.empty((N, K), dtype=torch.float32, device=device)
    db = torch.empty((N,), dtype=torch.float32, device=device) if want_db else None
    return dw, db, 0


def _wgrad(dy2, x2, mask, relu_x, want_db, out=None):
    M, N = dy2.shape
    K = x2.shape[1]
    L = lib()
    if _USE_X3 and M >= _X3_MIN_ROWS_WGRAD and L.nsdp_linear_wgrad_bf16x3_supported(_ll(M), _ci(N), _ci(K)):
        return _wgrad_x3(dy2, x2, mask, relu_x, want_db, out)
    L.nsdp_linear_wgrad_workspace_bytes.restype = ctypes.c_size_t
    nbytes = int(L.nsdp_linear_wgrad_workspace_bytes(_ll(M), _ci(N), _ci(K)))
    ws = torch.empty(max(nbytes // 4, 1), dtype=torch.float32, device=dy2.device)
    dw, db, acc = wgrad_out(out, N, K, want_db, dy2.device)
    batch = _cur_reduce
    if batch is not None and BATCH_REDUCE > 0 and M > 0:
        ptrs = {dw.data_ptr()} | ({db.data_ptr()} if db is not None else set())
        with on_device(dy2):
            if ptrs & batch["targets"]:
                _flush_reduce(batch)
            desc = _ReduceDescB16()
            check(L.nsdp_linear_wgrad_partials_f32(fptr(dy2, "dy"), fptr(x2, "x"), optptr(mask), _ci(int(relu_x)), fptr(dw),
                                                   optptr(db), _ll(M), _ci(N), _ci(K), _ci(acc), fptr(ws),
                                                   ctypes.c_size_t(nbytes), ctypes.byref(desc), stream_ptr()),
                  "nsdp_linear_wgrad_partials_f32")
            if desc.S == 0:
                return dw, db
            batch["descs_b16"].append(desc)
            batch["keep"].append((ws, dw, db))
            batch["targets"] |= ptrs
            if len(batch["descs"]) + len(batch["descs_b16"]) >= BATCH_REDUCE:
                _flush_reduce(batch)
        return dw, db
    with on_device(dy2):
        check(L.nsdp_linear_wgrad_f32(fptr(dy2, "dy"), fptr(x2, "x"), optptr(mask), _ci(int(relu_x)), fptr(dw),
                                      optptr(db), _ll(M), _ci(N), _ci(K), _ci(acc), fptr(ws),
                                      ctypes.c_size_t(nbytes), stream_ptr()), "nsdp_linear_wgrad_f32")
    return dw, db


class _ReduceDesc(ctypes.Structure):
    _fields_ = [("ws", ctypes.c_void_p), ("dW", ctypes.c_void_p), ("db", ctypes.c_void_p), ("S", ctypes.c_int),
                ("nta", ctypes.c_int), ("ktb", ctypes.c_int), ("N", ctypes.c_int), ("K", ctypes.c_int),
                ("accumulate", ctypes.c_int), ("reserved", ctypes.c_int)]


BATCH_REDUCE = int(os.environ.get("NSDP_WGRAD_BATCH_REDUCE", "16"))
_cur_reduce = None


class _ReduceDescB16(ctypes.Structure):
    _fields_ = [("ws", ctypes.c_void_p), ("dW", ctypes.c_void_p), ("db", ctypes.c_void_p), ("S", ctypes.c_int),
                ("N", ctypes.c_int), ("K", ctypes.c_int), ("accumulate", ctypes.c_int), ("reserved", ctypes.c_int)]


def _new_reduce_batch():
    return {"descs": [], "descs_b16": [], "keep": [], "targets": set()}


def _flush_reduce(batch):
    n = len(batch["descs"])
    if n:
        arr = (_ReduceDesc * n)(*batch["descs"])
        check(lib().nsdp_wgrad_bf16x3_reduce_batched(arr, _ci(n), stream_ptr()), "nsdp_wgrad_bf16x3_reduce_batched")
    n = len(batch["descs_b16"])
    if n:
        arr = (_ReduceDescB16 * n)(*batch["descs_b16"])
        check(lib().nsdp_wgrad_bf16_reduce_batched(arr, _ci(n), stream_ptr()), "nsdp_wgrad_bf16_reduce_batched")
    batch["descs"].clear()
    batch["descs_b16"].clear()
    batch["keep"].clear()
    batch["targets"].clear()


def _wgrad_x3(dy2, x2, mask, relu_x, want_db, out=None):
    M, N = dy2.shape
    K = x2.shape[1]
    L = lib()
    L.nsdp_linear_wgrad_bf16x3_workspace_bytes.restype = ctypes.c_size_t
    nbytes = int(L.nsdp_linear_wgrad_bf16x3_workspace_bytes(_ll(M), _ci(N), _ci(K)))
    ws = torch.empty(max(nbytes // 4, 1), dtype=torch.float32, device=dy2.device)
    dw, db, acc = wgrad_out(out, N, K, want_db, dy2.device)
    batch = _cur_reduce
    if batch is not None and BATCH_REDUCE > 0:
        ptrs = {dw.data_ptr()} | ({db.data_ptr()} if db is not None else set())
        if ptrs & batch["targets"]:
            with on_device(dy2):
                _flush_reduce(batch)
        desc = _ReduceDesc()
        with on_device(dy2):
            check(L.nsdp_linear_wgrad_bf16x3_partials_f32(fptr(dy2, "dy"), fptr(x2, "x"), optptr(mask), _ci(int(relu_x)), fptr(dw),
                                                          optptr(db), _ll(M), _ci(N), _ci(K), _ci(acc), fptr(ws),
                                                          ctypes.c_size_t(nbytes), ctypes.byref(desc), stream_ptr()),
                  "nsdp_linear_wgrad_bf16x3_partials_f32")
            batch["descs"].append(desc)
            batch["keep"].append((ws, dw, db))
            batch["targets"] |= ptrs
            if len(batch["descs"]) + len(batch["descs_b16"]) >= BATCH_REDUCE:
                _flush_reduce(batch)
        return dw, db
    with on_device(dy2):
        check(L.nsdp_linear_wgrad_bf16x3_f32(fptr(dy2, "dy"), fptr(x2, "x"), optptr(mask), _ci(int(relu_x)), fptr(dw),
                                             optptr(db), _ll(M), _ci(N), _ci(K), _ci(acc), fptr(ws),
                                             ctypes.c_size_t(nbytes), stream_ptr()), "nsdp_linear_wgrad_bf16x3_f32")
    return dw, db


_OVERLAP_WGRAD = os.environ.get("NSDP_WGRAD_STREAM", "auto")
_OVERLAP_WGRAD = {"0": False, "1": True}.get(_OVERLAP_WGRAD, "auto")
_OVERLAP_MIN_ROWS = 131072
SIDE_RESERVE_CUS = int(os.environ["NSDP_WGRAD_RESERVE_CUS"]) if "NSDP_WGRAD_RESERVE_CUS" in os.environ else None
_RESERVE_SMALL_ROWS = 131072
_reserve_now = {}
_overlap_now = {}
_side = {}
_pending = {}
_reduce_batches = {}


_graph_task_id = getattr(torch._C, "_current_graph_task_id", None)
_engine = getattr(torch.autograd.Variable, "_execution_engine", None)
_HAVE_ENGINE_HOOKS = _graph_task_id is not None and hasattr(_engine, "queue_callback")


def _pass_key(device):
    return (device.index, _graph_task_id())


def _side_stream(device):
    key = device.index
    if key not in _side:
        _side[key] = torch.cuda.Stream(device=device)
    return _side[key]


def _publish(device, key):
    _overlap_now.pop(key, None)
    _reserve_now.pop(key, None)
    todo = _pending.pop(key, {})
    batch = _reduce_batches.pop(key, None)
    if batch is not None and (batch["descs"] or batch["descs_b16"]):
        with torch.cuda.device(device), torch.cuda.stream(_side_stream(device)):
            _flush_reduce(batch)
    if not todo:
        return
    main = torch.cuda.current_stream(device)
    main.wait_stream(_side_stream(device))
    with torch.no_grad():
        for param, g in todo.values():
            if g is param.grad:
                continue
            g.record_stream(main)
            if param.grad is None:
                param.grad = g
            else:
                param.grad.add_(g)


def _wgrad_sliced(dy2, x2, mask, relu_x, want_db, k_orig, out=None):
    global _cur_reduce
    padded = x2.shape[1] != k_orig
    prev = _cur_reduce
    if padded:
        _cur_reduce = None
    try:
        dw, db = _wgrad(dy2, x2, mask, relu_x, want_db, None if padded else out)
    finally:
        _cur_reduce = prev
    if dw.shape[1] != k_orig:
        dw = dw[:, :k_orig].contiguous()
    return dw, db


REMASK_K4 = os.environ.get("NSDP_REMASK_K4", "1") != "0"


def _padded_w4(w_param, batch=True):
    key = _pack_key(w_param)
    hit = w_param.__dict__.get("_nsdp_w4")
    if hit is not None and hit[0] == key:
        return hit[1]
    w = w_param.detach()
    w = w.squeeze(-1) if w.dim() == 3 else w
    if w.shape[1] < 4 and w.is_contiguous() and w.is_cuda:
        reg = _pack_registry.get(w.device.index)
        ent = reg["entries"].get((id(w_param), "w4")) if reg is not None else None
        if (batch and hit is not None and ent is not None and ent[0]() is w_param and ent[2] is hit[1]
                and len(reg["entries"]) >= _BATCH_MIN and _repack_all(w.device)):
            return w_param.__dict__["_nsdp_w4"][1]
    w4 = (F.pad(w, (0, 4 - w.shape[1])) if w.shape[1] < 4 else w).contiguous()
    w_param.__dict__["_nsdp_w4"] = (key, w4)
    if w.shape[1] < 4 and w.is_contiguous() and w.is_cuda:
        reg = _pack_registry.setdefault(w.device.index, {"entries": {}, "array": None})
        reg["entries"][(id(w_param), "w4")] = [weakref.ref(w_param), "w4", w4, None]
        reg["array"] = None
    return w4


def _wgrad_k4_remask(w4, bias, k_orig):
    def fn(dy2, x2, mask, relu_x, want_db, out=None):
        M, N = dy2.shape
        L = lib()
        L.nsdp_linear_wgrad_workspace_bytes.restype = ctypes.c_size_t
        nbytes = int(L.nsdp_linear_wgrad_workspace_bytes(_ll(M), _ci(N), _ci(4)))
        ws = torch.empty(max(nbytes // 4, 1), dtype=torch.float32, device=dy2.device)
        dw = torch.empty((N, 4), dtype=torch.float32, device=dy2.device)
        db = torch.empty((N,), dtype=torch.float32, device=dy2.device) if want_db else None
        with on_device(dy2):
            check(L.nsdp_linear_wgrad_k4_remask_f32(fptr(dy2, "dy"), fptr(x2, "x"), fptr(w4, "weight"), optptr(bias), fptr(dw),
                                                    optptr(db), _ll(M), _ci(N), _ci(0), fptr(ws), ctypes.c_size_t(nbytes),
                                                    stream_ptr()), "nsdp_linear_wgrad_k4_remask_f32")
        return (dw[:, :k_orig].contiguous() if k_orig < 4 else dw), db
    return fn


def _grad_targets(w_param, b_param, gw, gb):
    if gw is None or (b_param is not None and gb is None) or not gw.is_contiguous():
        return None
    return gw.view(gw.shape[0], -1), gb


def wgrad_direct(dy2, x2, mask, relu_x, k_orig, w_param, b_param, fn=None):
    out = _grad_targets(w_param, b_param, w_param.grad, b_param.grad if b_param is not None else None)
    if fn is None:
        gw, gb = _wgrad_sliced(dy2, x2, mask, relu_x, b_param is not None, k_orig, out)
    else:
        gw, gb = fn(dy2, x2, mask, relu_x, b_param is not None, out)
    if out is not None and gw is out[0]:
        return
    with torch.no_grad():
        for prm, g in ((w_param, gw), (b_param, gb)):
            if prm is not None:
                g = g.view_as(prm)
                prm.grad = g if prm.grad is None else prm.grad.add_(g)


_last_decisions = {"overlap": None, "reserve": None}
_inherited = None


class inherit_pass_decisions:
    def __enter__(self):
        global _inherited
        self._was, _inherited = _inherited, dict(_last_decisions)
        return self

    def __exit__(self, *exc):
        global _inherited
        _inherited = self._was
        return False


def _use_side_stream(dy2):
    if not _HAVE_ENGINE_HOOKS:
        return False
    if _OVERLAP_WGRAD != "auto":
        return _OVERLAP_WGRAD
    key = _pass_key(dy2.device)
    use = _overlap_now.get(key)
    if use is None and _inherited is not None and _inherited["overlap"] is not None:
        use = _overlap_now[key] = _last_decisions["overlap"] = _inherited["overlap"]
        if not use:
            dev = dy2.device
            torch.autograd.Variable._execution_engine.queue_callback(lambda: _publish(dev, key))
    if use is None:
        use = _overlap_now[key] = dy2.shape[0] >= _OVERLAP_MIN_ROWS or torch.cuda.is_current_stream_capturing()
        _last_decisions["overlap"] = use
        if not use:
            dev = dy2.device
            torch.autograd.Variable._execution_engine.queue_callback(lambda: _publish(dev, key))
    return use


def _wgrad_deferred(dy2, x2, mask, relu_x, k_orig, w_param, b_param, fn=None):
    dev = dy2.device
    main = torch.cuda.current_stream(dev)
    side = _side_stream(dev)
    side.wait_stream(main)
    key = _pass_key(dev)
    slot = _pending.get(key)
    if slot is None:
        slot = _pending[key] = {}
        torch.autograd.Variable._execution_engine.queue_callback(lambda: _publish(dev, key))
    with torch.cuda.stream(side):
        ent_w = slot.get(id(w_param))
        ent_b = slot.get(id(b_param)) if b_param is not None else None
        if ent_w is None and (b_param is None or ent_b is None):
            gw0 = w_param.grad
            gb0 = b_param.grad if b_param is not None else None
            if gw0 is not None and (b_param is None or gb0 is not None):
                ent_w = slot[id(w_param)] = [w_param, gw0]
                if b_param is not None:
                    ent_b = slot[id(b_param)] = [b_param, gb0]
        out = _grad_targets(w_param, b_param, ent_w[1] if ent_w is not None else None, ent_b[1] if ent_b is not None else None)
        L = lib()
        reserve = _reserve_now.get(key)
        if reserve is None and _inherited is not None and _inherited["reserve"] is not None:
            reserve = _reserve_now[key] = _last_decisions["reserve"] = _inherited["reserve"]
        if reserve is None:
            reserve = _reserve_now[key] = (SIDE_RESERVE_CUS if SIDE_RESERVE_CUS is not None
                                           else (64 if dy2.shape[0] < _RESERVE_SMALL_ROWS else 48))
            _last_decisions["reserve"] = reserve
        L.nsdp_debug_set(_ci(9), _ci(reserve))
        global _cur_reduce
        batch = _reduce_batches.get(key)
        if batch is None:
            batch = _reduce_batches[key] = _new_reduce_batch()
        _cur_reduce = batch if (fn is None or getattr(fn, "batched_reduce", False)) else None
        if out is not None and batch["targets"] and (
                out[0].data_ptr() in batch["targets"] or (out[1] is not None and out[1].data_ptr() in batch["targets"])):
            _flush_reduce(batch)
        try:
            if fn is None:
                dw, db = _wgrad_sliced(dy2, x2, mask, relu_x, b_param is not None, k_orig, out)
            else:
                dw, db = fn(dy2, x2, mask, relu_x, b_param is not None, out)
        finally:
            _cur_reduce = None
            L.nsdp_debug_set(_ci(9), _ci(0))
        if out is None or dw is not out[0]:
            for param, g in ((w_param, dw), (b_param, db)):
                if param is None:
                    continue
                g = g.view_as(param)
                ent = slot.get(id(param))
                if ent is None:
                    slot[id(param)] = [param, g]
                else:
                    _flush_reduce(batch)
                    ent[1].add_(g)
    for t in (dy2, x2, mask) + tuple(getattr(fn, "extra_tensors", ())):
        if t is not None:
            t.record_stream(side)


def _pad_cols(t, mult=4):
    r = (-t.shape[-1]) % mult
    return t if r == 0 else F.pad(t, (0, r))


_USE_X3 = os.environ.get("NSDP_BF16X3", "1") != "0"
_X3_MIN_ROWS = int(os.environ.get("NSDP_X3_MIN_ROWS", "32768"))
_X3_MIN_ROWS_WGRAD = 2048


def _x3_ok(M, N, K):
    return _USE_X3 and M >= _X3_MIN_ROWS and K > 32 and K % 4 == 0 and N % 4 == 0 and N <= 256


_weights_epoch = 0


def invalidate_weight_packs():
    global _weights_epoch
    _weights_epoch += 1


def _pack_key(t):
    return (t.data_ptr(), t._version, _weights_epoch)


def _param_key(t):
    return (t.data_ptr(), t._version, t.__dict__.get("_nsdp_steps", 0))


def _after_optimizer_step(opt):
    invalidate_weight_packs()
    for group in opt.param_groups:
        for prm in group["params"]:
            prm.__dict__["_nsdp_steps"] = prm.__dict__.get("_nsdp_steps", 0) + 1


try:
    from torch.optim.optimizer import register_optimizer_step_post_hook as _reg_post_hook
    _reg_post_hook(lambda _opt, _args, _kwargs: _after_optimizer_step(_opt))
except ImportError:
    pass


class _PackDesc(ctypes.Structure):
    _fields_ = [("W", ctypes.c_void_p), ("Wp", ctypes.c_void_p), ("WpT", ctypes.c_void_p),
                ("N", ctypes.c_int), ("K", ctypes.c_int), ("kind", ctypes.c_int), ("reserved", ctypes.c_int)]


_pack_registry = {}
_BATCH_MIN = 8


def _repack_all(device):
    reg = _pack_registry[device.index]
    ents = reg["entries"]
    dead = [k for k, e in ents.items() if e[0]() is None]
    for k in dead:
        del ents[k]
        reg["array"] = None
    live = sorted(ents.values(), key=lambda e: e[1] == "b16")
    n_b16 = sum(1 for e in live if e[1] == "b16")
    if reg["array"] is None or len(reg["array"]) != len(live):
        reg["array"] = (_PackDesc * len(live))()
    arr = reg["array"]
    for i, (ref, kind, wp, wpt) in enumerate(live):
        prm = ref()
        w = prm.detach()
        w = w.squeeze(-1) if w.dim() == 3 else w
        if not w.is_contiguous():
            return False
        d = arr[i]
        d.W, d.Wp, d.WpT = w.data_ptr(), (wp.data_ptr() if wp is not None else None), (wpt.data_ptr() if wpt is not None else None)
        d.N, d.K, d.kind = w.shape[0], w.shape[1], {"wp": 0, "x3": 1, "b16": 2, "w4": 3}[kind]
    with torch.cuda.device(device):
        n_f = len(live) - n_b16
        if n_f:
            check(lib().nsdp_pack_weights_batched(arr, _ci(n_f), stream_ptr()), "nsdp_pack_weights_batched")
        if n_b16:
            tail = ctypes.cast(ctypes.byref(arr, n_f * ctypes.sizeof(_PackDesc)), ctypes.POINTER(_PackDesc))
            check(lib().nsdp_pack_weights_bf16(tail, _ci(n_b16), stream_ptr()), "nsdp_pack_weights_bf16")
    torch.autograd.graph.increment_version([t for e in live for t in e[2:4] if t is not None])
    for ref, kind, wp, wpt in live:
        prm = ref()
        if kind == "w4":
            prm.__dict__["_nsdp_w4"] = (_pack_key(prm), wp)
            continue
        cache = prm.__dict__.get("_nsdp_pack")
        key = _pack_key(prm)
        if cache is None or cache["key"] != key:
            cache = prm.__dict__["_nsdp_pack"] = {"key": key}
        cache[kind] = (wp, wpt)
    return True


def registered_packs(device):
    reg = _pack_registry.get(device.index if device.index is not None else torch.cuda.current_device())
    if reg is None:
        return []
    return [(ent[0](), ent[2], ent[3]) for ent in reg["entries"].values() if ent[0]() is not None]


def refresh_weight_packs(device):
    reg = _pack_registry.get(device.index)
    if reg is None or len(reg["entries"]) < _BATCH_MIN:
        return
    for ent in reg["entries"].values():
        prm = ent[0]()
        if prm is None:
            continue
        cache = prm.__dict__.get("_nsdp_pack")
        if cache is None or cache["key"] != _pack_key(prm):
            _repack_all(device)
            return


def _packs(w, owner, kind, want_t):
    cache = None
    if owner is not None:
        key = _pack_key(w)
        cache = owner.__dict__.get("_nsdp_pack")
        stale = cache is not None and cache["key"] != key
        if cache is None or stale:
            reg = _pack_registry.get(w.device.index)
            ent = reg["entries"].get((id(owner), kind)) if reg is not None else None
            if (stale and ent is not None and ent[0]() is owner and len(reg["entries"]) >= _BATCH_MIN
                    and (ent[3] is not None or not want_t) and _repack_all(w.device)):
                cache = owner.__dict__["_nsdp_pack"]
            else:
                cache = owner.__dict__["_nsdp_pack"] = {"key": key}
        ent = cache.get(kind)
        if ent is not None and (ent[1] is not None or not want_t):
            return ent
    wc = w if w.is_contiguous() else w.contiguous()
    if kind == "b16":
        from .hip_linear_bf16 import pack_weight_b16
        ent = pack_weight_b16(wc, True, want_t)
    else:
        ent = pack_weight_x3(wc, True, want_t) if kind == "x3" else pack_weight(wc, True, want_t)
    if cache is not None:
        cache[kind] = ent
        if wc is w:
            reg = _pack_registry.setdefault(w.device.index, {"entries": {}, "array": None})
            reg["entries"][(id(owner), kind)] = [weakref.ref(owner), kind, ent[0], ent[1]]
            reg["array"] = None
    return ent


def _run(kind, x2, pack, N, b, residual, mask, out_mask, relu_in, relu_out, res_sign=1.0, addend=None, lay=0, mask_bits=None,
         bits_out=None):
    if lay:
        if kind != "x3" or res_sign != 1.0:
            raise ValueError("G16 layouts belong to the bf16x3 kernels")
        return _fwd_x3_g16(x2, pack, N, b, residual, None if mask_bits is not None else mask, out_mask, relu_in, relu_out, lay,
                           addend=addend, mask_bits=mask_bits, bits_out=bits_out)
    if addend is not None:
        if kind == "x3" and mask is not None and out_mask is not None and not relu_in:
            return _fwd_x3(x2, pack, N, b, residual, mask, out_mask, relu_in, relu_out, addend=addend)
        return _run(kind, x2, pack, N, b, residual, mask, out_mask, relu_in, relu_out, res_sign).add_(addend)
    if res_sign != 1.0:
        if kind == "x3":
            return _fwd_x3(x2, pack, N, b, residual, mask, out_mask, relu_in, relu_out, res_sign)
        residual = -residual
    fn = _fwd_x3 if kind == "x3" else _fwd_wp
    return fn(x2, pack, N, b, residual, mask, out_mask, relu_in, relu_out)


class InputGradSum:
    __slots__ = ("total", "pending", "buf")

    def __init__(self):
        self.total = 0
        self.pending = 0
        self.buf = None


class SkipGrad:
    __slots__ = ("armed", "buf")

    def __init__(self):
        self.armed = False
        self.buf = None


K4_LINK = os.environ.get("NSDP_K4_LINK", "1") != "0"
K4_TAIL = os.environ.get("NSDP_K4_TAIL", "1") != "0"
K4_TAIL_SIDE = os.environ.get("NSDP_K4_TAIL_SIDE", "1") != "0"
K4_TAIL_RESERVE = int(os.environ["NSDP_K4_TAIL_RESERVE"]) if "NSDP_K4_TAIL_RESERVE" in os.environ else None


class K4Tail:
    __slots__ = ("armed", "taken", "x4", "w_param", "b_param", "k_orig", "fwd_key")

    def __init__(self):
        self.armed = self.taken = False
        self.x4 = self.w_param = self.b_param = self.k_orig = self.fwd_key = None


def _k4tail_fn(link, wpt, n_hidden, kind_t, h0):
    def fn(dy2, x4, mask, relu_x, want_db, out=None):
        M, K = dy2.shape
        L = lib()
        b0 = None if link.b_param is None else link.b_param.detach()
        if not (K4_TAIL and kind_t == "x3" and L.nsdp_linear_bf16x3_k4tail_ok(_ll(M), _ci(n_hidden), _ci(K))):
            dh = _run(kind_t, dy2, wpt, n_hidden, None, None, None, None, False, False)
            if REMASK_K4 and n_hidden % 4 == 0 and n_hidden >= 16 and M >= 4096:
                return _wgrad_k4_remask(_padded_w4(link.w_param, batch=False), b0, link.k_orig)(dh, x4, None, False, want_db, out)
            return _wgrad_sliced(dh, x4, h0, False, want_db, link.k_orig, out)
        L.nsdp_linear_bf16x3_k4tail_workspace_bytes.restype = ctypes.c_size_t
        nbytes = int(L.nsdp_linear_bf16x3_k4tail_workspace_bytes(_ll(M), _ci(n_hidden)))
        ws = torch.empty(max(nbytes // 4, 4), dtype=torch.float32, device=dy2.device)
        dw, db, acc = wgrad_out(out, n_hidden, link.k_orig, want_db, dy2.device)
        with on_device(dy2):
            if K4_TAIL_RESERVE is not None and torch.cuda.current_stream(dy2.device) == _side.get(dy2.device.index):
                L.nsdp_debug_set(_ci(9), _ci(K4_TAIL_RESERVE))
            check(L.nsdp_linear_bf16x3_k4tail_f32(fptr(dy2, "dy"), ctypes.c_void_p(wpt.data_ptr()), fptr(x4, "x4"),
                                                  fptr(_padded_w4(link.w_param, batch=False), "w0"), optptr(b0), fptr(dw), optptr(db), _ll(M),
                                                  _ci(n_hidden), _ci(K), _ci(int(link.k_orig)), _ci(acc), fptr(ws),
                                                  ctypes.c_size_t(nbytes), stream_ptr()), "nsdp_linear_bf16x3_k4tail_f32")
        return dw, db
    return fn


H0_RECOMPUTE = int(os.environ.get("NSDP_H0_RECOMPUTE", "1"))


def _h0_pays(M, N):
    nt = (N + 15) // 16
    if H0_RECOMPUTE >= 2 or nt <= 8:
        return True
    if nt <= 13:
        return M >= (1 << 19)
    return M <= 65536


def _fwd_x3_h0(x4, w4, b0, wp, N, K, b, gather):
    M = x4.shape[0]
    gq = gk = gidx = None
    g_div = rps = nsrc = 0
    if gather is not None:
        gq, g_div, gk, gidx, rps, nsrc = gather
        if (gq is not None and gq.shape[-1] != N) or gk.shape[-1] != N or gidx.numel() != M:
            raise ValueError("init_gather: table width / index count do not match the layer")
    y = torch.empty((M, N), dtype=torch.float32, device=x4.device)
    with on_device(x4):
        check(lib().nsdp_linear_bf16x3_h0_f32(fptr(x4, "x4"), fptr(w4, "w0"), optptr(b0), ctypes.c_void_p(wp.data_ptr()), optptr(b),
                                              optptr(gq), _ci(int(g_div)), optptr(gk),
                                              ctypes.c_void_p(gidx.data_ptr() if gidx is not None else None), _ci(int(rps)),
                                              _ci(int(nsrc)), fptr(y), _ll(M), _ci(N), _ci(K), stream_ptr()),
              "nsdp_linear_bf16x3_h0_f32")
    return y


def _wgrad_h0_fn(w4, b0, K):
    def fn(dy2, x4, mask, relu_x, want_db, out=None):
        M, N = dy2.shape
        L = lib()
        L.nsdp_linear_wgrad_bf16x3_workspace_bytes.restype = ctypes.c_size_t
        nbytes = int(L.nsdp_linear_wgrad_bf16x3_workspace_bytes(_ll(M), _ci(N), _ci(K)))
        ws = torch.empty(max(nbytes // 4, 1), dtype=torch.float32, device=dy2.device)
        dw, db, acc = wgrad_out(out, N, K, want_db, dy2.device)
        batch = _cur_reduce if BATCH_REDUCE > 0 else None
        desc = _ReduceDesc() if batch is not None else None
        with on_device(dy2):
            if batch is not None:
                ptrs = {dw.data_ptr()} | ({db.data_ptr()} if db is not None else set())
                if ptrs & batch["targets"]:
                    _flush_reduce(batch)
            check(L.nsdp_linear_wgrad_bf16x3_h0_f32(fptr(dy2, "dy"), fptr(x4, "x4"), fptr(w4, "w0"), optptr(b0), fptr(dw), optptr(db),
                                                    _ll(M), _ci(N), _ci(K), _ci(acc), fptr(ws), ctypes.c_size_t(nbytes),
                                                    ctypes.byref(desc) if desc is not None else None, stream_ptr()),
                  "nsdp_linear_wgrad_bf16x3_h0_f32")
            if batch is not None:
                batch["descs"].append(desc)
                batch["keep"].append((ws, dw, db, x4, w4, b0))
                batch["targets"] |= ptrs
                if len(batch["descs"]) + len(batch["descs_b16"]) >= BATCH_REDUCE:
                    _flush_reduce(batch)
        return dw, db
    fn.batched_reduce = True
    return fn


class _PosMlpFn(torch.autograd.Function):

    @staticmethod
    def forward(ctx, x4, w4, b0, w1, b1, wp, wpt, init_gather, k_orig0, w0_param, b0_param, w1_param, b1_param):
        N, K = w1.shape
        y = _fwd_x3_h0(x4, w4, b0, wp, N, K, b1, init_gather)
        ctx.save_for_backward(x4, w4, b0, wpt)
        ctx.params = (w0_param, b0_param, w1_param, b1_param)
        ctx.k_orig0, ctx.n_out, ctx.hidden = k_orig0, N, K
        ctx.fwd_key = (_param_key(w0_param), None if b0_param is None else _param_key(b0_param))
        return y

    @staticmethod
    def backward(ctx, dy):
        x4, w4, b0, wpt = ctx.saved_tensors
        w0_param, b0_param, w1_param, b1_param = ctx.params
        if ctx.fwd_key != (_param_key(w0_param), None if b0_param is None else _param_key(b0_param)):
            raise RuntimeError("position-encoding MLP: its first layer changed between forward and backward; the hidden tensor "
                               "is recomputed from the parameters (NSDP_H0_RECOMPUTE=0 keeps it)")
        N, K = ctx.n_out, ctx.hidden
        dy2 = dy.reshape(-1, N)
        dy2 = dy2 if dy2.is_contiguous() else dy2.contiguous()
        link = K4Tail()
        link.x4, link.w_param, link.b_param, link.k_orig = x4, w0_param, b0_param, ctx.k_orig0
        fn1 = _wgrad_h0_fn(w4, b0, K)
        tfn = _k4tail_fn(link, wpt, K, "x3", None)
        if _use_side_stream(dy2):
            _wgrad_deferred(dy2, x4, None, False, K, w1_param, b1_param, fn=fn1)
            if K4_TAIL_SIDE:
                _wgrad_deferred(dy2, x4, None, False, ctx.k_orig0, w0_param, b0_param, fn=tfn)
                wpt.record_stream(_side_stream(dy2.device))
            else:
                wgrad_direct(dy2, x4, None, False, ctx.k_orig0, w0_param, b0_param, fn=tfn)
        else:
            wgrad_direct(dy2, x4, None, False, K, w1_param, b1_param, fn=fn1)
            wgrad_direct(dy2, x4, None, False, ctx.k_orig0, w0_param, b0_param, fn=tfn)
        return (None,) * 13


def pos_mlp(x, weight0, bias0, weight1, bias1, init_gather=None):
    if not H0_RECOMPUTE or precision.is_bf16() or x.dtype is not torch.float32 or x.shape[-1] not in (3, 4):
        return None
    grad = torch.is_grad_enabled()
    if grad and x.requires_grad:
        return None
    w0 = weight0.squeeze(-1) if weight0.dim() == 3 else weight0
    w1 = weight1.squeeze(-1) if weight1.dim() == 3 else weight1
    N, K = w1.shape
    if w0.shape[0] != K or w0.shape[1] not in (3, 4) or w0.shape[1] > x.shape[-1] or not (weight0.is_leaf and weight1.is_leaf):
        return None
    M = x.numel() // x.shape[-1]
    L = lib()
    if not (_x3_ok(M, N, K) and L.nsdp_linear_bf16x3_h0_supported(_ll(M), _ci(N), _ci(K)) and _h0_pays(M, N)):
        return None
    needs = [p for p in (weight0, bias0, weight1, bias1) if p is not None and p.requires_grad]
    train = grad and bool(needs)
    if train:
        every = [p for p in (weight0, bias0, weight1, bias1) if p is not None]
        if (len(needs) != len(every) or not _PARAM_GRADS_DIRECT or any(_observed(p) or not p.is_leaf for p in every)
                or not (K4_LINK and REMASK_K4) or M < 4096 or not _x3_ok(M, K, N)
                or not L.nsdp_linear_wgrad_bf16x3_h0_supported(_ll(M), _ci(N), _ci(K))):
            return None
    x4 = x.reshape(-1, x.shape[-1])
    x4 = x4 if x4.is_contiguous() else x4.contiguous()
    x4 = _pad_cols(x4)
    w4 = _padded_w4(weight0)
    b0 = None if bias0 is None else bias0.detach()
    b1 = None if bias1 is None else bias1.detach()
    wd = w1.detach()
    wp = _packs(wd, weight1, "x3", train)[0]
    if not train:
        y = _fwd_x3_h0(x4, w4, b0, wp, N, K, b1, init_gather)
    else:
        wpt = _packs(wd, weight1, "x3", True)[1]
        y = _PosMlpFn.apply(x4, w4, b0, wd, b1, wp, wpt, init_gather, int(w0.shape[1]), weight0, bias0, weight1, bias1)
    return y.reshape(*x.shape[:-1], N)


class _LinearFn(torch.autograd.Function):
    @staticmethod
    def forward(ctx, x, w, b, residual, relu_in, relu_out, w_param=None, b_param=None, grad_sum=None, owner=None, bw=0,
                init_gather=None, res_sign=1.0, skip=None, tail=None, lay=0):
        ctx.lay = lay
        ctx.tail = None
        ctx.skip_src = ctx.skip_dst = None
        if skip is not None:
            link, is_src = skip
            if is_src:
                if residual is None or relu_out:
                    raise ValueError("skip_src: the layer that adds x as its residual, without an output ReLU")
                if link.armed and ctx.needs_input_grad[3]:
                    ctx.skip_src = link
            elif ctx.needs_input_grad[0]:
                if grad_sum is not None:
                    raise ValueError("skip_dst and InputGradSum do not combine")
                link.armed = True
                ctx.skip_dst = link
        ctx.premasked, ctx.mask_dx = bool(bw & 1) and relu_out, bool(bw & 2)
        ctx.w_param, ctx.b_param = w_param, b_param
        owner = w_param if w_param is not None else owner
        ctx.grad_sum = None
        if grad_sum is not None and ctx.needs_input_grad[0]:
            if relu_in or (bw & 2) or x.shape[-1] % 4:
                raise ValueError("InputGradSum: layers with a fused input ReLU or a padded input width cannot join")
            grad_sum.total += 1
            grad_sum.pending += 1
            ctx.grad_sum = grad_sum
        K = x.shape[-1]
        N = w.shape[0]
        if K != w.shape[1]:
            if not (K == 4 and w.shape[1] == 3) or ctx.needs_input_grad[0]:
                raise ValueError(f"linear: input width {K} against a [{N}, {w.shape[1]}] weight")
        x2 = x.reshape(-1, K)
        x2 = x2 if x2.is_contiguous() else x2.contiguous()
        K = w.shape[1]
        if K % 4 and x2.shape[1] % 4:
            x2 = _pad_cols(x2)
        res2 = None
        if residual is not None:
            res2 = residual.reshape(-1, N)
            res2 = res2 if res2.is_contiguous() else res2.contiguous()
        M, Kp = x2.shape
        want_t = bool(ctx.needs_input_grad[0])
        kind = "x3" if _x3_ok(M, N, Kp) else "wp"
        kind_t = "x3" if _x3_ok(M, Kp, N) else "wp"
        wp = _packs(w, owner, kind, want_t and kind_t == kind)[0]
        wpt = _packs(w, owner, kind_t, True)[1] if want_t else None
        if tail is not None:
            tlink, t_src = tail
            if t_src:
                if (not ctx.needs_input_grad[0] and w_param is not None and Kp == 4 and relu_out and not relu_in
                        and res2 is None and grad_sum is None and not bw and N % 4 == 0):
                    tlink.armed = True
                    tlink.x4, tlink.w_param, tlink.b_param, tlink.k_orig = x2, w_param, b_param, K
                    tlink.fwd_key = _param_key(w_param)
                    ctx.set_materialize_grads(False)
            elif (tlink.armed and want_t and not relu_in and not (bw & 2) and grad_sum is None and ctx.skip_dst is None
                  and Kp == K and N % 4 == 0 and M == tlink.x4.shape[0]):
                tlink.taken = True
                ctx.tail = tlink
        if lay and (kind != "x3" or init_gather is not None or bw or tail is not None or (lay == LAY_Y and res2 is not None)
                    or (lay == LAY_X and (grad_sum is not None or ctx.skip_dst is not None))):
            raise ValueError("G16 layout: a plain bf16x3 layer pair only (g16_pair_ok)")
        bits = None
        if init_gather is not None:
            if kind != "x3" or res2 is not None:
                raise ValueError("init_gather needs a layer on the bf16x3 kernel (gather_init_ok) without a residual")
            y = _fwd_x3_gather(x2, wp, N, b, init_gather, relu_in, relu_out)
        else:
            if (lay == LAY_Y and G16_BITS and relu_out and not ctx.premasked
                    and (ctx.needs_input_grad[0] or w_param is not None or ctx.needs_input_grad[1])):
                bits = relu_bits(M, N, x2.device)
            y = _run(kind, x2, wp, N, b, res2, None, None, relu_in, relu_out, res_sign, lay=lay, bits_out=bits)
        ctx.res_sign = res_sign
        ctx.relu_in, ctx.relu_out = relu_in, relu_out
        ctx.has_bias, ctx.has_res = b is not None, residual is not None
        ctx.x_shape, ctx.k_orig, ctx.n_out, ctx.kind_t = x.shape, K, N, kind_t
        ctx.fwd_key = _param_key(w_param) if w_param is not None else None
        ctx.save_for_backward(x2, wpt, y if (relu_out and not ctx.premasked and bits is None) else None, bits)
        return y.reshape(*x.shape[:-1], N)

    @staticmethod
    def backward(ctx, dy):
        if dy is None:
            return (None,) * 16
        x2, wpt, y, bits = ctx.saved_tensors
        N = ctx.n_out
        dy2 = dy.reshape(-1, N)
        dy2 = dy2 if dy2.is_contiguous() else dy2.contiguous()
        dx = dw = db = dres = None
        lay = ctx.lay
        if ctx.w_param is not None:
            fn = None
            if lay:
                fn = _wgrad_g16_fn(1 if lay == LAY_Y else 2, bits)
            elif (REMASK_K4 and y is not None and x2.shape[1] == 4 and not ctx.relu_in and N % 4 == 0 and N >= 16
                    and x2.shape[0] >= 4096 and not ctx.has_res and ctx.fwd_key == _param_key(ctx.w_param)):
                fn = _wgrad_k4_remask(_padded_w4(ctx.w_param, batch=False), None if ctx.b_param is None else ctx.b_param.detach(),
                                      ctx.k_orig)
            if _use_side_stream(dy2):
                _wgrad_deferred(dy2, x2, y, ctx.relu_in, ctx.k_orig, ctx.w_param, ctx.b_param, fn=fn)
            else:
                wgrad_direct(dy2, x2, y, ctx.relu_in, ctx.k_orig, ctx.w_param, ctx.b_param, fn=fn)
        elif ctx.needs_input_grad[1] or (ctx.has_bias and ctx.needs_input_grad[2]):
            if lay:
                dw, db = _wgrad_g16_fn(1 if lay == LAY_Y else 2, bits)(dy2, x2, y, ctx.relu_in, ctx.has_bias)
            else:
                dw, db = _wgrad_sliced(dy2, x2, y, ctx.relu_in, ctx.has_bias, ctx.k_orig)
        tl = ctx.tail
        if tl is not None and ctx.needs_input_grad[0] and tl.fwd_key == _param_key(tl.w_param):
            tfn = _k4tail_fn(tl, wpt, x2.shape[1], ctx.kind_t, x2)
            if K4_TAIL_SIDE and _use_side_stream(dy2):
                _wgrad_deferred(dy2, tl.x4, None, False, tl.k_orig, tl.w_param, tl.b_param, fn=tfn)
                wpt.record_stream(_side_stream(dy2.device))
            else:
                wgrad_direct(dy2, tl.x4, None, False, tl.k_orig, tl.w_param, tl.b_param, fn=tfn)
        elif ctx.needs_input_grad[0]:
            dyk, mk = dy2, y
            if N % 4:
                dyk = _pad_cols(dy2)
                mk = _pad_cols(y) if y is not None else None
            link = ctx.grad_sum
            addend = None
            if ctx.skip_dst is not None:
                addend, ctx.skip_dst.buf = ctx.skip_dst.buf, None
                if addend is not None and addend.shape[1] != x2.shape[1]:
                    raise RuntimeError("SkipGrad: the skip gradient does not have the layer's input width")
            dx = _run(ctx.kind_t, dyk, wpt, x2.shape[1], None, link.buf if link is not None else None, mk,
                      x2 if (ctx.relu_in or ctx.mask_dx) else None, False, False, addend=addend,
                      lay=(LAY_X if lay == LAY_Y else LAY_Y if lay == LAY_X else 0), mask_bits=bits)
            dx = dx[:, :ctx.k_orig].reshape(ctx.x_shape) if ctx.k_orig != dx.shape[1] else dx.reshape(ctx.x_shape)
            if link is not None:
                link.pending -= 1
                if link.pending > 0:
                    link.buf, dx = dx.reshape(-1, ctx.k_orig), None
                else:
                    link.buf, link.pending = None, link.total
        if ctx.skip_src is not None:
            ctx.skip_src.buf = dy2
        elif ctx.has_res and ctx.needs_input_grad[3]:
            dres = dy2 if y is None else dy2 * (y > 0)
            dres = dres.reshape(dy.shape)
            if ctx.res_sign != 1.0:
                dres = -dres
        return dx, dw, db, dres, None, None, None, None, None, None, None, None, None, None, None, None


_PARAM_GRADS_DIRECT = os.environ.get("NSDP_PARAM_GRADS", "direct") != "autograd"


class autograd_param_grads:

    def __enter__(self):
        global _PARAM_GRADS_DIRECT
        self._was, _PARAM_GRADS_DIRECT = _PARAM_GRADS_DIRECT, False
        return self

    def __exit__(self, *exc):
        global _PARAM_GRADS_DIRECT
        _PARAM_GRADS_DIRECT = self._was
        return False


def _observed(t):
    return bool(t._backward_hooks) or bool(getattr(t, "_post_accumulate_grad_hooks", None))


def linear(x, weight, bias=None, relu_in=False, relu_out=False, residual=None, params=False, grad_sum=None,
           out_f32=False, premasked=False, mask_dx=False, init_gather=None, residual_sign=1.0,
           skip_src=None, skip_dst=None, tail_src=None, tail_dst=None, pack_owner=None, lay=0):
    bw = (1 if premasked else 0) | (2 if mask_dx else 0)
    w_param = b_param = None
    if (params and _PARAM_GRADS_DIRECT and torch.is_grad_enabled() and weight.requires_grad and weight.is_leaf
            and not _observed(weight)):
        w_param = weight
        b_param = bias if (bias is not None and bias.requires_grad and bias.is_leaf) else None
        if bias is not None and (b_param is None or _observed(bias)):
            w_param = b_param = None
    w2 = weight.squeeze(-1) if weight.dim() == 3 else weight
    owner = weight if (params and weight.is_leaf) else None
    if pack_owner is not None:
        owner = pack_owner
    if precision.is_bf16():
        if init_gather is not None or residual_sign != 1.0 or skip_src or skip_dst or lay:
            raise ValueError("init_gather / signed residuals / SkipGrad / G16 layouts belong to fp32 storage")
        if bw:
            raise ValueError("premasked / mask_dx belong to fp32 storage (bf16 storage uses relu_in on the second layer)")
        from . import hip_linear_bf16 as hb
        K, N = x.shape[-1], w2.shape[0]
        if (hb.NATIVE and x.dtype is torch.bfloat16 and 8 <= K <= 256 and K % 8 == 0 and N <= 256
                and (out_f32 or N % 4 == 0)):
            if residual is not None and residual.dtype is not torch.bfloat16:
                residual = residual.to(torch.bfloat16)
            return hb.linear(x, weight, bias, relu_in, relu_out, residual, w_param, b_param, grad_sum, owner, out_f32)
        if hb.NATIVE and not out_f32 and grad_sum is None and hb.k4_supported(x, N, relu_in, residual):
            return hb.linear_k4(x, weight, bias, relu_out, w_param, b_param)
        if grad_sum is not None and hb.NATIVE:
            raise ValueError("InputGradSum needs a bf16 layer in bf16 storage mode")
        xf = x if x.dtype is torch.float32 else x.float()
        rf = residual if (residual is None or residual.dtype is torch.float32) else residual.float()
        if w_param is not None:
            y = _LinearFn.apply(xf, w2.detach(), None if bias is None else bias.detach(), rf, bool(relu_in),
                                bool(relu_out), w_param, b_param, grad_sum)
        else:
            y = _LinearFn.apply(xf, w2, bias, rf, bool(relu_in), bool(relu_out), None, None, grad_sum, owner)
        return y if out_f32 else y.to(torch.bfloat16)
    if skip_src is not None and skip_dst is not None:
        raise ValueError("a layer is either end of a SkipGrad link")
    skip = (skip_src, True) if skip_src is not None else (skip_dst, False) if skip_dst is not None else None
    tail = (tail_src, True) if tail_src is not None else (tail_dst, False) if tail_dst is not None else None
    if w_param is not None:
        return _LinearFn.apply(x, w2.detach(), None if bias is None else bias.detach(), residual, bool(relu_in),
                               bool(relu_out), w_param, b_param, grad_sum, None, bw, init_gather,
                               float(residual_sign), skip, tail, int(lay))
    return _LinearFn.apply(x, w2, bias, residual, bool(relu_in), bool(relu_out), None, None, grad_sum, owner, bw,
                           init_gather, float(residual_sign), skip, None, int(lay))
```

nsdp_amd/model/decoder/blocks.py:

```python
from __future__ import annotations

import os

import torch
import torch.nn as nn
import torch.nn.functional as F

from .. import ops
from ... import precision


PREFETCH_RESERVE_CUS = int(os.environ.get("NSDP_PREFETCH_RESERVE_CUS", "0"))


class CrossTransformerBlock(nn.Module):

    def __init__(self, dim_inp, dim, nneigh=7, reduce_dim=True, separate_delta=True):
        super().__init__()
        self.dim = dim
        self.nneigh = nneigh
        self.separate_delta = separate_delta
        self.fc_delta = nn.Sequential(nn.Linear(3, dim), nn.ReLU(), nn.Linear(dim, dim))
        self.fc_gamma = nn.Sequential(nn.Linear(dim, dim), nn.ReLU(), nn.Linear(dim, dim))
        self.w_k_global = nn.Linear(dim_inp, dim, bias=False)
        self.w_v_global = nn.Linear(dim_inp, dim, bias=False)
        self.w_qs = nn.Linear(dim_inp, dim, bias=False)
        self.w_ks = nn.Linear(dim_inp, dim, bias=False)
        self.w_vs = nn.Linear(dim_inp, dim, bias=False)
        if not reduce_dim:
            self.fc = nn.Linear(dim, dim_inp)
        self.reduce_dim = reduce_dim

    def prefetch(self, xyz_q, xyz, after=None):
        from ... import hip_linear
        hip_linear.refresh_weight_packs(xyz_q.device)
        main = torch.cuda.current_stream(xyz_q.device)
        s = ops.prefetch_stream(xyz_q.device)
        s.wait_stream(main)
        if after is not None:
            s.wait_stream(after)
        with torch.cuda.stream(s):
            idx = ops.knn_indices(xyz_q, xyz, self.nneigh)
            rel = ops.relative_coords(xyz_q, xyz, idx)
            hip_linear.lib().nsdp_debug_set(9, PREFETCH_RESERVE_CUS)
            try:
                pos = ops.mlp2(rel, self.fc_delta)
            finally:
                hip_linear.lib().nsdp_debug_set(9, 0)
        return {"xyz_q": xyz_q, "xyz": xyz, "idx": idx, "rel": rel, "pos": pos, "stream": s}

    def forward(self, xyz_q, lat_rep, xyz, points, prefetched=None, idx=None):
        assert lat_rep.dim() == 2, "per-query latent codes are not used by any NSDP configuration"
        pos = None
        if prefetched is not None and prefetched["xyz_q"] is xyz_q and prefetched["xyz"] is xyz:
            main = torch.cuda.current_stream(xyz_q.device)
            main.wait_stream(prefetched["stream"])
            idx, rel, pos = prefetched["idx"], prefetched["rel"], prefetched["pos"]
            for t in (idx, rel, pos):
                t.record_stream(main)
        elif idx is None:
            idx = ops.knn_indices(xyz_q, xyz, self.nneigh)
        q = ops.linear(lat_rep, self.w_qs)
        k_g = ops.linear(lat_rep, self.w_k_global)
        v_g = ops.linear(lat_rep, self.w_v_global)
        kf = ops.linear(points, self.w_ks)
        vf = ops.linear(points, self.w_vs)
        if pos is None:
            rel = ops.relative_coords(xyz_q, xyz, idx)
        logit_g = ops.mlp2(q - k_g, self.fc_gamma)
        res, _ = ops.vector_attention(rel, q.unsqueeze(1), kf, vf, idx, self.fc_delta,
                                      self.fc_gamma, a_g=logit_g, v_g=v_g, pos=pos)
        if not self.reduce_dim:
            res = ops.linear(res, self.fc)
        return res


class ResnetBlockFC(nn.Module):

    def __init__(self, size_in, size_out=None, size_h=None):
        super().__init__()
        size_out = size_in if size_out is None else size_out
        size_h = min(size_in, size_out) if size_h is None else size_h
        self.size_in, self.size_h, self.size_out = size_in, size_h, size_out
        self.fc_0 = nn.Linear(size_in, size_h)
        self.fc_1 = nn.Linear(size_h, size_out)
        self.shortcut = None if size_in == size_out else nn.Linear(size_in, size_out, bias=False)
        nn.init.zeros_(self.fc_1.weight)

    def forward(self, x):
        x_s = x if self.shortcut is None else ops.linear(x, self.shortcut)
        if precision.is_bf16():
            h = ops.linear(x, self.fc_0, relu_in=True)
            return ops.linear(h, self.fc_1, relu_in=True, residual=x_s)
        pair = ops.PAIR_MASK and torch.is_grad_enabled()
        skip = ops.skip_grad(x) if self.shortcut is None else None
        g16 = not pair and ops.g16_pair(x, self.fc_0, self.fc_1, relu_in0=True)
        h = ops.linear(x, self.fc_0, relu_in=True, relu=True, premasked=pair, skip_dst=skip,
                       lay=ops.hip_linear.LAY_Y if g16 else 0)
        return ops.linear(h, self.fc_1, residual=x_s, mask_dx=pair, skip_src=skip,
                          lay=ops.hip_linear.LAY_X if g16 else 0)
```

nsdp_amd/model/decoder/crosstransformer_decoder.py:

```python
from __future__ import annotations

import torch
import torch.nn as nn

from .. import ops
from ... import hip_decoder, hip_linear, precision
from ...ragged import RaggedPoints
from .blocks import CrossTransformerBlock, ResnetBlockFC

TRUNK_F32 = __import__("os").environ.get("NSDP_BF16_TRUNK", "bf16") == "f32"


class CrossTransformerDecoder(nn.Module):

    def __init__(self, dim_inp, dim, nneigh=7, hidden_dim=64, n_blocks=5, out_dim=1):
        super().__init__()
        self.dim = dim
        self.n_blocks = n_blocks
        self.ct1 = CrossTransformerBlock(dim_inp, dim, nneigh=nneigh)
        self.init_enc = nn.Linear(dim, hidden_dim)
        self.blocks = nn.ModuleList([ResnetBlockFC(hidden_dim) for _ in range(n_blocks)])
        self.fc_c = nn.ModuleList([nn.Linear(dim, hidden_dim) for _ in range(n_blocks)])
        self.fc_out = nn.Linear(hidden_dim, out_dim)

    def prefetch(self, xyz_q, anchors, after=None):
        if isinstance(xyz_q, RaggedPoints):
            return None
        if hip_decoder.fused_for_inference() and not torch.is_grad_enabled() and hip_decoder.supported(self):
            return None
        return self.ct1.prefetch(xyz_q, anchors, after)

    @staticmethod
    def _query_idx(xyz_q, encoding):
        return encoding.get("query_idx") if encoding.get("query_points") is xyz_q else None

    @torch.no_grad()
    def geometry(self, xyz_q, anchors):
        return {"query_idx": ops.knn_indices(xyz_q, anchors, self.ct1.nneigh)}

    def forward(self, xyz_q, encoding):
        if isinstance(xyz_q, RaggedPoints):
            return hip_decoder.decoder_forward_ragged(self, xyz_q, encoding)
        if hip_decoder.fused_for_inference() and not torch.is_grad_enabled() and hip_decoder.supported(self):
            return hip_decoder.decoder_forward(self, xyz_q, encoding)
        lat = self.ct1(xyz_q, encoding["z"], encoding["anchors"], encoding["anchor_feats"], prefetched=encoding.get("prefetch"),
                       idx=self._query_idx(xyz_q, encoding))
        if precision.is_bf16() and TRUNK_F32:
            with precision.storage(torch.float32):
                return self._trunk(lat.float())
        return self._trunk(lat)

    def _trunk(self, lat):
        fan = hip_linear.InputGradSum() if (torch.is_grad_enabled() and lat.requires_grad) else None
        net = ops.linear(lat, self.init_enc, grad_sum=fan)
        for i in range(self.n_blocks):
            net = ops.linear(lat, self.fc_c[i], residual=net, grad_sum=fan)
            net = self.blocks[i](net)
        return ops.linear(net, self.fc_out, relu_in=True, out_f32=True)
```

nsdp_amd/model/ops.py:

```python
from __future__ import annotations

import os

import torch
import torch.nn as nn
import torch.nn.functional as F

from .. import hip_attention, hip_batchnorm, hip_linear, precision
from .. import pointnet2_utils as pu


_GEOMETRY_ABLATE = os.environ.get("NSDP_GEOMETRY_ABLATE", "0") == "1"
_ablate_cache = {}


@torch.no_grad()
def knn_indices(query: torch.Tensor, source: torch.Tensor, k: int) -> torch.Tensor:
    if _GEOMETRY_ABLATE:
        key = ("knn", tuple(query.shape), tuple(source.shape), k)
        if key not in _ablate_cache:
            _ablate_cache[key] = pu.knn(query.detach().contiguous(), source.detach().contiguous(), k)
        return _ablate_cache[key]
    return pu.knn(query.detach().contiguous(), source.detach().contiguous(), k)


@torch.no_grad()
def fps_indices(xyz: torch.Tensor, npoint: int) -> torch.Tensor:
    return pu.furthest_point_sample(xyz.detach().contiguous(), npoint)


def attention_lists(idx: torch.Tensor, n: int, N: int, d: int, per_shape_query: bool = False):
    if not hip_attention._use_inverse(torch.float32, per_shape_query, n, N, d):
        return None
    return hip_attention.inverse_lists(idx, N)


_side_streams = {}
PYRAMID_LISTS = os.environ.get("NSDP_PYRAMID_LISTS", "1") != "0"


def _side_stream(device):
    key = (device.type, device.index)
    if key not in _side_streams:
        _side_streams[key] = torch.cuda.Stream(device=device)
    return _side_streams[key]


def geometry_stream(device):
    return _side_streams.get((device.type, device.index))


_prefetch_streams = {}


def prefetch_stream(device):
    key = (device.type, device.index)
    if key not in _prefetch_streams:
        _prefetch_streams[key] = torch.cuda.Stream(device=device)
    return _prefetch_streams[key]


@torch.no_grad()
def geometry_pyramid(xyz: torch.Tensor, npoints, ks, overlap: bool = True, dims=None):
    if _GEOMETRY_ABLATE:
        key = ("pyramid", tuple(xyz.shape), tuple(npoints), tuple(ks), None if dims is None else tuple(dims))
        if key in _ablate_cache:
            return _ablate_cache[key], (lambda: None)
    main = torch.cuda.current_stream(xyz.device)
    side = _side_stream(xyz.device) if overlap else main
    if overlap:
        side.wait_stream(main)
    levels = []
    with torch.cuda.stream(side):
        cur = xyz.detach().contiguous()
        for n_new, (k_sa, k_blk) in zip(npoints, ks):
            fps_idx = pu.furthest_point_sample(cur, n_new)
            new_xyz = pu.gather_rows(cur, fps_idx)
            sa_idx = pu.knn(new_xyz, cur, k_sa)
            blk_idx = pu.knn(new_xyz, new_xyz, k_blk) if k_blk is not None else None
            lv = {"fps_idx": fps_idx, "new_xyz": new_xyz, "sa_idx": sa_idx, "blk_idx": blk_idx}
            if dims is not None and PYRAMID_LISTS:
                d = dims[len(levels)]
                if hip_attention._use_inverse(torch.float32, False, n_new, cur.shape[1], d):
                    lv["sa_inv"] = hip_attention.inverse_lists(sa_idx, cur.shape[1])
                if blk_idx is not None and hip_attention._use_inverse(torch.float32, False, n_new, n_new, d):
                    lv["blk_inv"] = hip_attention.inverse_lists(blk_idx, n_new)
            levels.append(lv)
            cur = new_xyz

    if _GEOMETRY_ABLATE and not torch.cuda.is_current_stream_capturing():
        _ablate_cache[key] = levels

    def join():
        if overlap:
            torch.cuda.current_stream(xyz.device).wait_stream(side)
            for lv in levels:
                for t in lv.values():
                    for u in (t if isinstance(t, tuple) else (t,)):
                        if u is not None:
                            u.record_stream(torch.cuda.current_stream(xyz.device))

    return levels, join


class _GatherRows(torch.autograd.Function):

    @staticmethod
    def forward(ctx, points, idx):
        B, N, C = points.shape
        flat = idx.reshape(B, -1)
        ctx.save_for_backward(flat)
        ctx.n = N
        points = points.contiguous()
        if points.dtype is torch.bfloat16 and C % 2 == 0:
            out = pu.gather_rows(points.view(torch.float32), flat).view(torch.bfloat16)
        else:
            out = pu.gather_rows(points.float(), flat).to(points.dtype)
        return out.reshape(*idx.shape, C)

    @staticmethod
    def backward(ctx, grad_out):
        (flat,) = ctx.saved_tensors
        B = flat.shape[0]
        g = grad_out.reshape(B, flat.shape[1], -1).contiguous()
        if g.dtype is torch.bfloat16:
            return pu.scatter_add_rows(g.float(), flat, ctx.n).to(torch.bfloat16), None
        return pu.scatter_add_rows(g, flat, ctx.n), None


def index_points(points: torch.Tensor, idx: torch.Tensor) -> torch.Tensor:
    return _GatherRows.apply(points, idx)


REL4 = os.environ.get("NSDP_REL4", "1") != "0"


def relative_coords(query: torch.Tensor, source: torch.Tensor, idx: torch.Tensor, sign: float = 1.0) -> torch.Tensor:
    if (REL4 and query.is_cuda and query.dtype is torch.float32 and source.dtype is torch.float32 and idx.dim() == 3
            and not (torch.is_grad_enabled() and (query.requires_grad or source.requires_grad))):
        return pu.rel_coords4(query.detach().contiguous(), source.detach().contiguous(), idx.contiguous(), sign)
    d = query.unsqueeze(2) - index_points(source, idx)
    return d if sign > 0 else -d


def linear(x: torch.Tensor, lin, relu: bool = False, relu_in: bool = False, residual=None, grad_sum=None,
           out_f32: bool = False, premasked: bool = False, mask_dx: bool = False,
           init_gather=None, residual_sign: float = 1.0, skip_src=None, skip_dst=None, tail_src=None,
           tail_dst=None, lay: int = 0) -> torch.Tensor:
    return hip_linear.linear(x, lin.weight, lin.bias, relu_in=relu_in, relu_out=relu, residual=residual,
                             params=True, grad_sum=grad_sum, out_f32=out_f32, premasked=premasked, mask_dx=mask_dx,
                             init_gather=init_gather, residual_sign=residual_sign,
                             skip_src=skip_src, skip_dst=skip_dst, tail_src=tail_src, tail_dst=tail_dst, lay=lay)


def g16_pair(x: torch.Tensor, lin0, lin1, relu_in0: bool = False) -> bool:
    if not (hip_linear.G16 and x.is_cuda and x.dtype is torch.float32) or precision.is_bf16():
        return False
    K = x.shape[-1]
    w0 = lin0.weight.squeeze(-1) if lin0.weight.dim() == 3 else lin0.weight
    w1 = lin1.weight.squeeze(-1) if lin1.weight.dim() == 3 else lin1.weight
    if w0.shape[1] != K or w1.shape[1] != w0.shape[0]:
        return False
    train = torch.is_grad_enabled() and (x.requires_grad or lin0.weight.requires_grad or lin1.weight.requires_grad)
    return hip_linear.g16_pair_ok(x.numel() // K, K, w0.shape[0], w1.shape[0], relu_in0=relu_in0, train=train)


def pos_mlp(x: torch.Tensor, seq: nn.Sequential, init_gather=None):
    if PAIR_MASK:
        return None
    return hip_linear.pos_mlp(x, seq[0].weight, seq[0].bias, seq[2].weight, seq[2].bias, init_gather=init_gather)


def k4_tail(x: torch.Tensor, seq: nn.Sequential):
    if (hip_linear.K4_LINK and torch.is_grad_enabled() and not x.requires_grad and not precision.is_bf16() and not PAIR_MASK
            and x.shape[-1] in (3, 4) and seq[0].weight.requires_grad):
        return hip_linear.K4Tail()
    return None


def input_grad_sum(x: torch.Tensor):
    return hip_linear.InputGradSum() if (torch.is_grad_enabled() and x.requires_grad) else None


PAIR_MASK = os.environ.get("NSDP_PAIR_MASK", "0") == "1"


def mlp2(x: torch.Tensor, seq: nn.Sequential, grad_sum=None) -> torch.Tensor:
    if precision.is_bf16():
        return linear(linear(x, seq[0], grad_sum=grad_sum), seq[2], relu_in=True)
    if PAIR_MASK and torch.is_grad_enabled():
        return linear(linear(x, seq[0], relu=True, grad_sum=grad_sum, premasked=True), seq[2], mask_dx=True)
    if grad_sum is None and x.shape[-1] in (3, 4):
        y = pos_mlp(x, seq)
        if y is not None:
            return y
    tl = k4_tail(x, seq) if grad_sum is None else None
    g16 = tl is None and g16_pair(x, seq[0], seq[2])
    return linear(linear(x, seq[0], relu=True, grad_sum=grad_sum, tail_src=tl, lay=hip_linear.LAY_Y if g16 else 0), seq[2],
                  tail_dst=tl, lay=hip_linear.LAY_X if g16 else 0)


def batch_norm(x: torch.Tensor, bn: nn.BatchNorm1d, addend=None, relu: bool = False) -> torch.Tensor:
    if x.dtype is torch.bfloat16 and not hip_batchnorm.NATIVE_BF16:
        a = None if addend is None else addend.float()
        return hip_batchnorm.batch_norm(x.float(), bn, addend=a, relu=relu).to(torch.bfloat16)
    return hip_batchnorm.batch_norm(x, bn, addend=addend, relu=relu)


SKIP_GRAD = os.environ.get("NSDP_SKIP_GRAD", "1") != "0"


def skip_grad(x):
    if SKIP_GRAD and torch.is_grad_enabled() and x.requires_grad and not precision.is_bf16():
        return hip_linear.SkipGrad()
    return None


FUSE_DPOS = os.environ.get("NSDP_FUSE_DPOS", "1") != "0"
FUSE_PRE = os.environ.get("NSDP_FUSE_PRE", "1") != "0"


class PosAsU:
    __slots__ = ("y", "q", "kf")

    def __init__(self, y, q, kf):
        self.y, self.q, self.kf = y, q, kf


COMBINE_TABLES = os.environ.get("NSDP_COMBINE_TABLES", "1") != "0"


def fused_pre_applies(idx, d) -> bool:
    B, n, k = idx.shape
    return bool(FUSE_PRE and COMBINE_TABLES and not precision.is_bf16() and not PAIR_MASK and hip_linear.gather_init_ok(B * n * k, d, d))


def vector_attention(rel, q, kf, vf, idx, fc_delta, fc_gamma, residual=None, pos=None, a_g=None, v_g=None, combined=False,
                     inv=None):
    if isinstance(pos, PosAsU):
        y, q1, k1 = pos.y, pos.q, pos.kf
        link = hip_attention.pos_grad_link() if y.requires_grad else None
        if link is not None and FUSE_DPOS:
            link.grad_sum = hip_linear.InputGradSum()
        inv = inv if inv is not None else hip_attention.backward_lists(idx, y.shape[1], kf.shape[1], y.shape[-1])
        u = hip_attention.attn_pre(q, kf, y, idx, link, inv) if combined else hip_attention.attn_pre(q - q1, kf - k1, y, idx, link, inv)
        logits = mlp2(u, fc_gamma, grad_sum=link.grad_sum if link is not None else None)
        out = hip_attention.attn_post(logits, vf, y, idx, a_g=a_g, v_g=v_g, residual=residual, link=link, inv=inv,
                                      sub=(None if combined else k1, q1))
        return out, pos
    if (pos is None and q is not None and FUSE_PRE and not precision.is_bf16() and not PAIR_MASK
            and hip_linear.gather_init_ok(rel.shape[0] * rel.shape[1] * rel.shape[2], fc_delta[2].weight.shape[0],
                                          fc_delta[2].weight.shape[1])):
        B, n, k = idx.shape
        d = fc_delta[2].weight.shape[0]
        per_shape = q.shape[1] == 1 and n != 1
        qd, kd = q.detach(), kf.detach()
        if per_shape:
            gather = (None, 1, (qd - kd).reshape(-1, d), idx.reshape(-1), n * k, kf.shape[1])
        else:
            gather = (qd.reshape(-1, d).contiguous(), k, kd.reshape(-1, d).contiguous(), idx.reshape(-1), n * k, kf.shape[1])
        y = pos_mlp(rel, fc_delta, init_gather=gather)
        if y is None:
            tl = k4_tail(rel, fc_delta)
            h = linear(rel, fc_delta[0], relu=True, tail_src=tl)
            y = linear(h, fc_delta[2], init_gather=gather, tail_dst=tl)
        link = hip_attention.pos_grad_link() if y.requires_grad else None
        if link is not None and FUSE_DPOS:
            link.grad_sum = hip_linear.InputGradSum()
        inv = inv if inv is not None else hip_attention.backward_lists(idx, n, kf.shape[1], d, qb=per_shape)
        u = hip_attention.attn_pre(q, kf, y, idx, link, inv, precomputed=y.detach())
        logits = mlp2(u, fc_gamma, grad_sum=link.grad_sum if link is not None else None)
        out = hip_attention.attn_post(logits, vf, y, idx, a_g=a_g, v_g=v_g, residual=residual, link=link, inv=inv,
                                      sub=(None if combined else kd, qd))
        return out, PosAsU(y, qd, kd)
    if combined:
        raise ValueError("combined tables were prepared for the fused path (fused_pre_applies), which this call does not take")
    if pos is None:
        pos = mlp2(rel, fc_delta)
    if q is None:
        logits = mlp2(pos, fc_gamma)
        out = hip_attention.attn_post(logits, None, pos, idx, residual=residual)
    else:
        link = hip_attention.pos_grad_link() if pos.requires_grad else None
        if link is not None and FUSE_DPOS and hip_attention.native(pos):
            link.grad_sum = hip_linear.InputGradSum()
        if inv is None:
            inv = hip_attention.backward_lists(idx, pos.shape[1], kf.shape[1], pos.shape[-1], qb=(q.shape[1] == 1 and pos.shape[1] != 1))
        u = hip_attention.attn_pre(q, kf, pos, idx, link, inv)
        logits = mlp2(u, fc_gamma, grad_sum=link.grad_sum if link is not None else None)
        out = hip_attention.attn_post(logits, vf, pos, idx, a_g=a_g, v_g=v_g, residual=residual, link=link, inv=inv)
    return out, pos
```

Baseline: 7.128 million query-points/s.

## Fuse consecutive linear layers into one K-segmented GEMM in decoder trunk

Adds a segmented-K variant of the bf16x3 linear kernel that accumulates several (X, W, bias) segments into one output tile in a single launch. The decoder trunk now fuses each resnet block's second linear with the next fc_c conditioning linear (and init_enc with fc_c[0]), so the intermediate residual is never written and re-read and launches drop. Backward is extended to return gradients for the extra segment. This adds per-iteration segment-cursor bookkeeping and bias injection inside the K loop, and the fused path is restricted to specific N and K shapes.

Result: faster. 7.265 million query-points/s, median of 6 (+1.9%).

```diff
diff --git a/include/nsdp_hip.h b/include/nsdp_hip.h
--- a/include/nsdp_hip.h
+++ b/include/nsdp_hip.h
@@ -103,6 +103,17 @@
 int nsdp_linear_bf16x3_f32(const float *X, const void *Wp, const float *bias, const float *residual,
                            const float *mask, const float *out_mask, float *Y, long long M, int N, int K,
                            int relu_in, int relu_out, void *stream);
+
+typedef struct {
+  const float *X;
+  const void *Wp;
+  const float *bias;
+  int K;
+  int layout;
+} NsdpLinearSeg;
+int nsdp_linear_bf16x3_seg_supported(long long M, int N, int nseg);
+int nsdp_linear_bf16x3_seg_f32(const NsdpLinearSeg *segs, int nseg, const float *residual, float *Y, long long M, int N,
+                               void *stream);
 
 int nsdp_linear_bf16x3_gather_f32(const float *X, const void *Wp, const float *bias, const float *gq, int g_div, const float *gk,
                                   const int32_t *gidx, int g_rows_per_shape, int g_nsrc, float *Y, long long M, int N, int K,
diff --git a/nsdp_amd/build.py b/nsdp_amd/build.py
--- a/nsdp_amd/build.py
+++ b/nsdp_amd/build.py
@@ -25,6 +25,7 @@
     "wgrad_bf16x3.hip": FAST + ["-O2", "-fno-slp-vectorize"],
     "gemm_bf16x3.hip": FAST + ["-fno-slp-vectorize"],
     "gemm_bf16x3_g16.hip": FAST + ["-fno-slp-vectorize"],
+    "gemm_bf16x3_seg.hip": FAST + ["-fno-slp-vectorize"],
 }
 
 
diff --git a/nsdp_amd/csrc/gemm_bf16x3_seg.hip b/nsdp_amd/csrc/gemm_bf16x3_seg.hip
--- /dev/null
+++ b/nsdp_amd/csrc/gemm_bf16x3_seg.hip
@@ -0,0 +1,59 @@
+#include "x3_kernel.h"
+
+#include "../../include/nsdp_hip.h"
+
+namespace {
+
+int seg_tiles(int N) {
+  return N == 128 ? 8 : N == 200 ? 13 : 0;
+}
+
+}
+
+extern "C" {
+
+int nsdp_linear_bf16x3_seg_supported(long long M, int N, int nseg) {
+  return M > 0 && M * 832 < (1LL << 32) && seg_tiles(N) != 0 && nseg >= 1 && nseg <= kMaxSeg;
+}
+
+int nsdp_linear_bf16x3_seg_f32(const NsdpLinearSeg *segs, int nseg, const float *residual, float *Y, long long M, int N,
+                               void *stream) {
+  if (M <= 0 || N <= 0) return 0;
+  NSDP_REQUIRE(segs && Y, "linear_bf16x3_seg: null pointer");
+  NSDP_REQUIRE(nsdp_linear_bf16x3_seg_supported(M, N, nseg), "linear_bf16x3_seg: unsupported call M=%lld N=%d segments=%d", M, N, nseg);
+  NSDP_REQUIRE(((reinterpret_cast<uintptr_t>(Y) | reinterpret_cast<uintptr_t>(residual)) & 15) == 0,
+               "linear_bf16x3_seg: all operands must be 16-byte aligned");
+  X3SegParams p{};
+  p.residual = residual;
+  p.Y = Y;
+  p.M = M;
+  p.N = N;
+  p.res_sign = 1.f;
+  p.nseg = nseg;
+  long long ksum = 0;
+  for (int s = 0; s < nseg; ++s) {
+    const NsdpLinearSeg &g = segs[s];
+    NSDP_REQUIRE(g.X && g.Wp, "linear_bf16x3_seg: segment %d: null pointer", s);
+    NSDP_REQUIRE(g.K > 32 && g.K % 4 == 0 && g.K <= 208, "linear_bf16x3_seg: segment %d: K=%d must be a multiple of 4 in (32, 208]", s, g.K);
+    NSDP_REQUIRE(g.layout == 0 || (g.layout == 1 && M % 16 == 0), "linear_bf16x3_seg: segment %d: layout %d (0 row-major, 1 G16 with M %% 16 == 0)",
+                 s, g.layout);
+    NSDP_REQUIRE(g.layout == 0 || seg_tiles(N) == 8, "linear_bf16x3_seg: segment %d: G16 segments come with N = 128 only", s);
+    NSDP_REQUIRE(!g.bias || s == nseg - 1 || seg_tiles(N) == 8,
+                 "linear_bf16x3_seg: segment %d: with N = 200 only the last segment may carry a bias", s);
+    NSDP_REQUIRE(((reinterpret_cast<uintptr_t>(g.X) | reinterpret_cast<uintptr_t>(g.Wp) | reinterpret_cast<uintptr_t>(g.bias)) & 15) == 0,
+                 "linear_bf16x3_seg: segment %d: operands must be 16-byte aligned", s);
+    p.seg[s] = X3Seg{g.X, g.Wp, g.bias, g.K, g.layout};
+    ksum += g.K;
+  }
+  for (int s = nseg; s < kMaxSeg; ++s) p.seg[s] = X3Seg{nullptr, nullptr, nullptr, 0, 0};
+  p.bias = segs[nseg - 1].bias;
+  p.K = static_cast<int>(ksum);
+  hipStream_t st = nsdp::as_stream(stream);
+  nsdp::prof::Scope scope(nsdp::prof::kLinearX3, st, 2.0 * M * N * ksum,
+                          4.0 * (static_cast<double>(M) * (ksum + N + (residual ? N : 0)) + static_cast<double>(N) * ksum));
+  if (seg_tiles(N) == 8) launch_x3_pre<2, 8, 0, 4, false, 2, 0, 0, true>(p, st, 2);
+  else launch_x3_pre<2, 13, 0, 4, true, 2, 0, 0, true>(p, st, 2);
+  return nsdp::launch_status("linear_bf16x3_kernel (seg)");
+}
+
+}
diff --git a/nsdp_amd/csrc/x3_kernel.h b/nsdp_amd/csrc/x3_kernel.h
--- a/nsdp_amd/csrc/x3_kernel.h
+++ b/nsdp_amd/csrc/x3_kernel.h
@@ -55,6 +55,18 @@
   const float *h_x4 = nullptr, *h_w0 = nullptr, *h_b0 = nullptr;
   const unsigned char *bits = nullptr;
   unsigned char *bits_out = nullptr;
+};
+
+struct X3Seg {
+  const float *X;
+  const void *Wp;
+  const float *bias;
+  int K, g16;
+};
+constexpr int kMaxSeg = 8;
+struct X3SegParams : X3Params {
+  int nseg = 0;
+  X3Seg seg[kMaxSeg];
 };
 
 constexpr int kLayX = 1;
@@ -123,6 +135,9 @@
 __device__ __forceinline__ void xload(f32x4 &dst, const float *lane_ptr) {
   asm volatile("global_load_dwordx4 %0, %1, off" : "=v"(dst) : "v"(lane_ptr));
 }
+__device__ __forceinline__ void xload_s(f32x4 &dst, unsigned lane_byte_off, const float *uniform_base) {
+  asm volatile("global_load_dwordx4 %0, %1, %2" : "=v"(dst) : "v"(lane_byte_off), "s"(uniform_base));
+}
 __device__ __forceinline__ void bload(unsigned &dst, const unsigned char *lane_ptr) {
   asm volatile("global_load_ubyte %0, %1, off" : "=v"(dst) : "v"(lane_ptr));
 }
@@ -151,8 +166,9 @@
   *reinterpret_cast<f32x4 *>(reinterpret_cast<char *>(uniform_base) + byte_off) = v;
 }
 
-template <int MT, int NT, int PRE, int WV, bool XREG = false, int KBM = 2, int GATHER = 0, int TAIL = 0, int LAY = 0>
-__global__ __launch_bounds__(WV * 64, XREG ? 2 : 1) void linear_bf16x3_kernel(X3Params p) {
+template <int MT, int NT, int PRE, int WV, bool XREG = false, int KBM = 2, int GATHER = 0, int TAIL = 0, int LAY = 0, bool SEG = false>
+__global__ __launch_bounds__(WV * 64, XREG ? 2 : 1) void linear_bf16x3_kernel(std::conditional_t<SEG, X3SegParams, X3Params> p) {
+  static_assert(!SEG || (PRE == 0 && !GATHER && !TAIL && !LAY && KBM == 2), "K segments: plain prologue, streaming weights, row-major Y");
   constexpr bool kXG = (LAY & kLayX) != 0, kYG = (LAY & kLayY) != 0, kRG = (LAY & kLayR) != 0;
   static_assert(!kYG || (!GATHER && !TAIL), "G16 output: plain epilogue forms");
   static_assert(!kXG || PRE != 3, "G16 input: there is no X in the H0 forms");
@@ -197,7 +213,18 @@
   const int wave = __builtin_amdgcn_readfirstlane(threadIdx.x >> 6);
   const int li = lane & 15, g = lane >> 4;
   const int K = p.K, N = p.N;
-  const int KB = (K + 31) >> 5;
+  const int dbg = SEG ? 0 : p.dbg;
+  int KB = (K + 31) >> 5;
+  struct SegCur { int s, k; };
+  auto seg_adv = [&](SegCur &c) {
+    if constexpr (SEG) {
+      if (++c.k >= ((p.seg[c.s].K + 31) >> 5)) { c.k = 0; if (++c.s >= p.nseg) c.s = 0; }
+    }
+  };
+  if constexpr (SEG) {
+    KB = 0;
+    for (int s = 0; s < p.nseg; ++s) KB += (p.seg[s].K + 31) >> 5;
+  }
   const int ntiles = (N + 15) >> 4;
   constexpr long long kRowsWg = static_cast<long long>(WV) * MT * 16;
   const long long wg_tiles = (p.M + kRowsWg - 1) / kRowsWg;
@@ -218,8 +245,10 @@
         m[mt] = reinterpret_cast<const float *>(p.bits + (r >> 4) * (static_cast<long long>((K + 31) >> 5) * 64) + (r & 15) * 4 + g);
     }
   };
-  set_rows(tile, xa, ma);
-  set_rows(tile + stride, xn, mn);
+  if constexpr (!SEG) {
+    set_rows(tile, xa, ma);
+    set_rows(tile + stride, xn, mn);
+  }
   f32x4 h_xs[kH0 ? MT : 1];
   int h_kb = 0;
   unsigned h_par = 0;
@@ -248,6 +277,15 @@
       __builtin_amdgcn_global_load_lds((gbl_ptr_t)(wlane + ((static_cast<long long>(kb) * pieces + q) << 10)),
                                        (lds_ptr_t)(wbuf_at(buf) + q * 64), 16, 0, 0);
   };
+  auto stage_seg = [&](SegCur c, int buf) {
+    if constexpr (SEG) {
+      const char *wl = static_cast<const char *>(p.seg[c.s].Wp) + lane * 16;
+      const int pieces = ntiles * 3;
+      for (int q = wave; q < pieces; q += WV)
+        __builtin_amdgcn_global_load_lds((gbl_ptr_t)(wl + ((static_cast<long long>(c.k) * pieces + q) << 10)),
+                                         (lds_ptr_t)(wbuf_at(buf) + q * 64), 16, 0, 0);
+    }
+  };
   const unsigned lds0 = static_cast<unsigned>(reinterpret_cast<uintptr_t>((lds_ptr_t)(&wlds[lane])));
   const unsigned ldsw = static_cast<unsigned>(reinterpret_cast<uintptr_t>((lds_ptr_t)(&wlds[0])));
   const unsigned ldsb = static_cast<unsigned>(reinterpret_cast<uintptr_t>((lds_ptr_t)(&bias_lds[0])));
@@ -267,7 +305,7 @@
         if constexpr (kXG) ko *= 16;
         if constexpr (kXLds) {
           const float *src = x[mt] + ko;
-          if (p.dbg & 1024) src = x[0] - li * K + (((kb * MT * 2 + mt * 2 + hf) * 256) % 6144) + lane * 4;
+          if (dbg & 1024) src = x[0] - li * K + (((kb * MT * 2 + mt * 2 + hf) * 256) % 6144) + lane * 4;
           __builtin_amdgcn_global_load_lds((gbl_ptr_t)src, (lds_ptr_t)(&xbuf[xb][wave][(mt * 2 + hf) * 64]), 16, 0, 0);
         } else {
           xload(raw[mt][hf], x[mt] + ko);
@@ -277,6 +315,28 @@
           }
         }
       }
+  };
+  auto xissue_seg = [&](long long t, SegCur c, unsigned xb) {
+    if constexpr (SEG) {
+      const float *sx = p.seg[c.s].X;
+      const unsigned sk = static_cast<unsigned>(p.seg[c.s].K);
+      const bool sg = !XREG && p.seg[c.s].g16 != 0;
+      const unsigned r0 = static_cast<unsigned>((t * WV + wave) * (MT * 16)), rmax = static_cast<unsigned>(p.M - 1);
+#pragma unroll
+      for (int mt = 0; mt < MT; ++mt) {
+        unsigned r = r0 + static_cast<unsigned>(mt * 16 + li);
+        r = r < rmax ? r : rmax;
+        const unsigned ro = (sg ? (r & ~15u) : r) * sk + (sg ? (r & 15u) * 4u : 0u);
+#pragma unroll
+        for (int hf = 0; hf < 2; ++hf) {
+          unsigned ko = static_cast<unsigned>(c.k * 32 + 16 * hf + 4 * g);
+          ko = ko < sk ? ko : (sk - 4u);
+          ko *= sg ? 16u : 1u;
+          if constexpr (kXLds) __builtin_amdgcn_global_load_lds((gbl_ptr_t)(sx + (ro + ko)), (lds_ptr_t)(&xbuf[xb][wave][(mt * 2 + hf) * 64]), 16, 0, 0);
+          else xload_s(raw[mt][hf], (ro + ko) * 4u, sx);
+        }
+      }
+    }
   };
   auto xwait = [&]() {
     if constexpr (kXLds || kH0) {
@@ -352,20 +412,31 @@
     if (WV == 4 && gridDim.x > 256 && blockIdx.x >= gridDim.x / 2) phase = (phase + 4) & 7;
     for (int i = 0; i < phase * KB; ++i) __builtin_amdgcn_s_sleep(10);
   }
-  if constexpr (WRES) {
-    for (int kb = 0; kb < KB; ++kb) stage(kb, kb);
+  SegCur cc{0, 0}, cw{0, 0}, cx{0, 0};
+  seg_adv(cw);
+  cx = cw;
+  seg_adv(cx);
+  if constexpr (SEG) {
+    stage_seg(cc, 0);
+    xissue_seg(tile, cc, 0u);
+    if constexpr (kXLds) xissue_seg(tile, cw, 1u);
   } else {
-    stage(0, 0);
-  }
-  xissue(xa, ma, 0, 0u);
-  if constexpr (kXLds) xissue(xa, ma, 1, 1u);
+    if constexpr (WRES) {
+      for (int kb = 0; kb < KB; ++kb) stage(kb, kb);
+    } else {
+      stage(0, 0);
+    }
+    xissue(xa, ma, 0, 0u);
+    if constexpr (kXLds) xissue(xa, ma, 1, 1u);
+  }
   xwait();
 #pragma unroll
   for (int mt = 0; mt < MT; ++mt)
 #pragma unroll
     for (int pr = 0; pr < 4; ++pr) convert_pair(cur, mt, pr, 0u);
   if constexpr (!kXLds) {
-    xissue(xa, ma, 1, 0u);
+    if constexpr (SEG) xissue_seg(tile, cw, 0u);
+    else xissue(xa, ma, 1, 0u);
     xwait();
   }
   __syncthreads();
@@ -434,10 +505,19 @@
       const unsigned buf = gs & 1u;
       const bool more = kb + 1 < KB || next_tile;
       if constexpr (!WRES) {
-        if (more && !(p.dbg & 1)) stage(kb + 1 < KB ? kb + 1 : 0, buf ^ 1u);
+        if constexpr (SEG) {
+          if (more) stage_seg(cw, buf ^ 1u);
+        } else {
+          if (more && !(dbg & 1)) stage(kb + 1 < KB ? kb + 1 : 0, buf ^ 1u);
+        }
       }
       bool x_issued = false;
-      if constexpr (kXLds) {
+      if constexpr (kXLds && SEG) {
+        if (kb + 2 < KB || next_tile) {
+          xissue_seg(kb + 2 < KB ? tile : tile + stride, cx, buf);
+          x_issued = true;
+        }
+      } else if constexpr (kXLds) {
         if (kb + 2 < KB) { xissue(xa, ma, kb + 2, buf); x_issued = true; }
         else if (next_tile) { xissue(xn, mn, kb + 2 - KB, buf); x_issued = true; }
       }
@@ -460,7 +540,7 @@
         u32x4 nh, nm, nl;
         if constexpr (nt + 1 < NT) {
           lds_read<(nt + 1) * 3072>(nh, wl_addr);
-          if (!(p.dbg & 512)) {
+          if (!(dbg & 512)) {
             lds_read<(nt + 1) * 3072 + 1024>(nm, wl_addr);
             lds_read<(nt + 1) * 3072 + 2048>(nl, wl_addr);
           } else {
@@ -468,8 +548,12 @@
           }
         }
         if constexpr (!kXLds && !kH0 && nt == kConvFirst + kConvSteps) {
-          if (kb + 2 < KB) xissue(xa, ma, kb + 2, 0u);
-          else if (next_tile) xissue(xn, mn, kb + 2 - KB, 0u);
+          if constexpr (SEG) {
+            if (kb + 2 < KB || next_tile) xissue_seg(kb + 2 < KB ? tile : tile + stride, cx, 0u);
+          } else {
+            if (kb + 2 < KB) xissue(xa, ma, kb + 2, 0u);
+            else if (next_tile) xissue(xn, mn, kb + 2 - KB, 0u);
+          }
         }
         if constexpr (kXLds && nt == kConvFirst) xwait_older();
         if constexpr (nt >= kConvFirst && nt < kConvFirst + kConvSteps) {
@@ -526,18 +610,48 @@
       asm volatile("" ::: "memory");
       X3_T(t_k3);
       X3_ADD(0, t_k0, t_k1); X3_ADD(1, t_k1, t_k2); X3_ADD(2, t_k2, t_k3);
+      if constexpr (SEG) {
+        if (cw.k == 0 && kb + 1 < KB) {
+          if constexpr (XREG) {
+          } else {
+            const float *sb = p.seg[cc.s].bias;
+            int g_b = g;
+            asm volatile("" : "+v"(g_b));
+            auto add_bias = [&](auto has_bias) {
+              static_for<0, NT>([&](auto I) {
+                constexpr int nt = decltype(I)::value;
+                f32x4 bv = {0.f, 0.f, 0.f, 0.f};
+                if constexpr (decltype(has_bias)::value) {
+                  const int col = nt * 16 + 4 * g_b;
+                  bv = *reinterpret_cast<const f32x4 *>(sb + (col + 4 <= N ? col : (N - 4)));
+                }
+#pragma unroll
+                for (int mt = 0; mt < MT; ++mt) {
+                  acc[mt][nt] += bv;
+                  asm volatile("" : "+a"(acc[mt][nt]));
+                }
+              });
+            };
+            if (sb) add_bias(std::true_type{});
+            else add_bias(std::false_type{});
+          }
+        }
+        cc = cw;
+        cw = cx;
+        seg_adv(cx);
+      }
       cur = nxt;
     }
 
     X3_T(t_e0);
-    if (row0 < p.M && !(p.dbg & 8)) {
+    if (row0 < p.M && !(dbg & 8)) {
       const bool full_rows = row0 + MT * 16 <= p.M;
       int li_e = li, g_e = g;
       asm volatile("" : "+v"(li_e), "+v"(g_e));
       float4 bias4[NT];
 #pragma unroll
       for (int nt = 0; nt < NT; ++nt) bias4[nt] = make_float4(0.f, 0.f, 0.f, 0.f);
-      if (p.bias && (!kStage || (p.dbg & (8192 | 16384 | 32768)))) {
+      if (p.bias && (!kStage || (dbg & (8192 | 16384 | 32768)))) {
 #pragma unroll
         for (int nt = 0; nt < NT; ++nt) {
           const int col = nt * 16 + 4 * g_e;
@@ -582,12 +696,12 @@
           const f32x4 vv = {v.x, v.y, v.z, v.w};
           if (decltype(guarded)::value) {
             if (cv && rv) {
-              if (p.dbg & 64) __builtin_nontemporal_store(vv, reinterpret_cast<f32x4 *>(p.Y + rowc * N + colc));
+              if (dbg & 64) __builtin_nontemporal_store(vv, reinterpret_cast<f32x4 *>(p.Y + rowc * N + colc));
               else *reinterpret_cast<f32x4 *>(p.Y + rowc * N + colc) = vv;
             }
           } else {
-            if (p.dbg & 64) __builtin_nontemporal_store(vv, reinterpret_cast<f32x4 *>(p.Y + row * N + col));
-            else if (p.dbg & 2048)
+            if (dbg & 64) __builtin_nontemporal_store(vv, reinterpret_cast<f32x4 *>(p.Y + row * N + col));
+            else if (dbg & 2048)
               *reinterpret_cast<f32x4 *>(p.Y + row0 * N + (((mt * NT + nt) * 256) % 6144) + (li_e + 16 * g_e) * 4) = vv;
             else *reinterpret_cast<f32x4 *>(p.Y + row * N + col) = vv;
           }
@@ -818,7 +932,7 @@
     tile += stride;
 #pragma unroll
     for (int mt = 0; mt < MT; ++mt) { xa[mt] = xn[mt]; ma[mt] = mn[mt]; }
-    set_rows(tile + stride, xn, mn);
+    if constexpr (!SEG) set_rows(tile + stride, xn, mn);
     if constexpr (kH0) {
       h_rows(tile + stride, h_par);
       h_par ^= 1u;
@@ -831,18 +945,18 @@
 #endif
 }
 
-template <int MT, int NT, int PRE, int WV, bool XREG = false, int KBM = 2, int GATHER = 0, int LAY = 0>
-void launch_x3_pre(const X3Params &p, hipStream_t st, int wgs_per_cu = 1) {
+template <int MT, int NT, int PRE, int WV, bool XREG = false, int KBM = 2, int GATHER = 0, int LAY = 0, bool SEG = false>
+void launch_x3_pre(const std::conditional_t<SEG, X3SegParams, X3Params> &p, hipStream_t st, int wgs_per_cu = 1) {
   const long long rows_per_wg = static_cast<long long>(WV) * MT * 16;
   const long long wg_tiles = (p.M + rows_per_wg - 1) / rows_per_wg;
   static const int reserve_env = getenv("NSDP_X3_RESERVE_CUS") ? atoi(getenv("NSDP_X3_RESERVE_CUS")) : 0;
   const int reserve = g_x3_side_reserve > 0 && g_x3_side_reserve < nsdp::num_cus() ? g_x3_side_reserve : reserve_env;
   const long long slots = static_cast<long long>(nsdp::num_cus() - reserve) * wgs_per_cu;
   const unsigned grid = static_cast<unsigned>(wg_tiles < slots ? wg_tiles : slots);
-  NSDP_TRACE("linear_bf16x3<%d,%d,%d,%d,%d>x%d%s%s%s", MT, NT, PRE, WV, static_cast<int>(XREG), wgs_per_cu, KBM > 2 ? " wres" : "",
-             GATHER == 2 ? " gather1" : GATHER ? " gather" : "",
+  NSDP_TRACE("linear_bf16x3<%d,%d,%d,%d,%d>x%d%s%s%s%s", MT, NT, PRE, WV, static_cast<int>(XREG), wgs_per_cu, KBM > 2 ? " wres" : "",
+             GATHER == 2 ? " gather1" : GATHER ? " gather" : "", SEG ? " seg" : "",
              LAY == 0 ? "" : LAY == 1 ? " g16:x" : LAY == 2 ? " g16:y" : LAY == 3 ? " g16:xy" : LAY == 4 ? " g16:r" : LAY == 5 ? " g16:xr" : LAY == 6 ? " g16:yr" : " g16:xyr");
-  hipLaunchKernelGGL((linear_bf16x3_kernel<MT, NT, PRE, WV, XREG, KBM, GATHER, 0, LAY>), dim3(grid), dim3(WV * 64), 0, st, p);
-}
-
-}
+  hipLaunchKernelGGL((linear_bf16x3_kernel<MT, NT, PRE, WV, XREG, KBM, GATHER, 0, LAY, SEG>), dim3(grid), dim3(WV * 64), 0, st, p);
+}
+
+}
diff --git a/nsdp_amd/hip_linear.py b/nsdp_amd/hip_linear.py
--- a/nsdp_amd/hip_linear.py
+++ b/nsdp_amd/hip_linear.py
@@ -128,6 +128,51 @@
                                                ctypes.c_void_p(mask_bits.data_ptr() if mask_bits is not None else None),
                                                ctypes.c_void_p(bits_out.data_ptr() if bits_out is not None else None), stream_ptr()),
               "nsdp_linear_bf16x3_g16_f32")
+    return y
+
+
+SEG_DX = os.environ.get("NSDP_SEG_DX", "1") != "0"
+SEG_FWD = os.environ.get("NSDP_SEG_FWD", "1") != "0"
+SEG_MAX = 8
+
+
+class _LinearSeg(ctypes.Structure):
+    _fields_ = [("X", ctypes.c_void_p), ("Wp", ctypes.c_void_p), ("bias", ctypes.c_void_p), ("K", ctypes.c_int),
+                ("layout", ctypes.c_int)]
+
+
+def seg_ok(M, N, ks, g16=False, inner_bias=False):
+    if precision.is_bf16() or not 1 <= len(ks) <= SEG_MAX or not all(_x3_ok(M, N, k) and k <= 208 for k in ks):
+        return False
+    if (g16 and M % 16) or ((g16 or inner_bias) and N != 128):
+        return False
+    return bool(lib().nsdp_linear_bf16x3_seg_supported(_ll(M), _ci(N), _ci(len(ks))))
+
+
+def seg_pair_ok(x, w, xe, we, fused_extras=False, lay=0, bias=True):
+    if fused_extras or lay not in (0, LAY_X) or w.dim() != 2 or we.dim() != 2 or w.shape[0] != we.shape[0]:
+        return False
+    if not (x.is_cuda and x.dtype is torch.float32 and xe.dtype is torch.float32):
+        return False
+    K, Ke, N = x.shape[-1], xe.shape[-1], w.shape[0]
+    if K != w.shape[1] or Ke != we.shape[1] or x.numel() // K != xe.numel() // Ke:
+        return False
+    return seg_ok(x.numel() // K, N, [K, Ke], g16=lay == LAY_X, inner_bias=bias)
+
+
+def _fwd_x3_seg(segs, N, residual=None):
+    M = segs[0][0].shape[0]
+    y = torch.empty((M, N), dtype=torch.float32, device=segs[0][0].device)
+    arr = (_LinearSeg * len(segs))()
+    for i, (x2, wp, b, g16) in enumerate(segs):
+        if x2.shape[0] != M:
+            raise ValueError("segments of one launch have the same rows")
+        arr[i].X, arr[i].Wp = fptr(x2, "x").value, wp.data_ptr()
+        arr[i].bias = b.data_ptr() if b is not None else None
+        arr[i].K, arr[i].layout = x2.shape[1], 1 if g16 else 0
+    with on_device(y):
+        check(lib().nsdp_linear_bf16x3_seg_f32(arr, _ci(len(segs)), optptr(residual), fptr(y), _ll(M), _ci(N), stream_ptr()),
+              "nsdp_linear_bf16x3_seg_f32")
     return y
 
 
@@ -705,12 +750,34 @@
 
 
 class InputGradSum:
-    __slots__ = ("total", "pending", "buf")
+    __slots__ = ("total", "pending", "buf", "segs")
 
     def __init__(self):
         self.total = 0
         self.pending = 0
         self.buf = None
+        self.segs = []
+
+    def flush(self, K):
+        if self.segs:
+            segs, self.segs = self.segs, []
+            self.buf = _fwd_x3_seg(segs, K, self.buf)
+        return self.buf
+
+
+def _plain_dx(link, kind_t, dyk, wpt, K):
+    if link is not None and link.total > 1 and SEG_DX and kind_t == "x3" and seg_ok(dyk.shape[0], K, [dyk.shape[1]]):
+        link.segs.append((dyk, wpt, None, False))
+        dx = link.flush(K) if (link.pending == 1 or len(link.segs) == SEG_MAX) else None
+    else:
+        dx = _run(kind_t, dyk, wpt, K, None, link.flush(K) if link is not None else None, None, None, False, False)
+    if link is not None:
+        link.pending -= 1
+        if link.pending > 0:
+            link.buf, dx = (dx if dx is not None else link.buf), None
+        else:
+            link.buf, link.pending = None, link.total
+    return dx
 
 
 class SkipGrad:
@@ -901,7 +968,7 @@
 class _LinearFn(torch.autograd.Function):
     @staticmethod
     def forward(ctx, x, w, b, residual, relu_in, relu_out, w_param=None, b_param=None, grad_sum=None, owner=None, bw=0,
-                init_gather=None, res_sign=1.0, skip=None, tail=None, lay=0):
+                init_gather=None, res_sign=1.0, skip=None, tail=None, lay=0, xe=None, we=None, be=None, extra=None):
         ctx.lay = lay
         ctx.tail = None
         ctx.skip_src = ctx.skip_dst = None
@@ -964,7 +1031,29 @@
                     or (lay == LAY_X and (grad_sum is not None or ctx.skip_dst is not None))):
             raise ValueError("G16 layout: a plain bf16x3 layer pair only (g16_pair_ok)")
         bits = None
-        if init_gather is not None:
+        ctx.extra = None
+        xe2 = wpte = None
+        if xe is not None:
+            if (kind != "x3" or relu_in or relu_out or init_gather is not None or bw or tail is not None or res_sign != 1.0
+                    or lay == LAY_Y):
+                raise ValueError("a second segment joins a plain bf16x3 layer only (seg_pair_ok)")
+            w_param_e, b_param_e, grad_sum_e, owner_e = extra
+            owner_e = w_param_e if w_param_e is not None else owner_e
+            Ke = we.shape[1]
+            xe2 = xe.reshape(-1, Ke)
+            xe2 = xe2 if xe2.is_contiguous() else xe2.contiguous()
+            want_te = bool(ctx.needs_input_grad[16])
+            kind_te = "x3" if _x3_ok(M, Ke, N) else "wp"
+            wpe = _packs(we, owner_e, "x3", want_te and kind_te == "x3")[0]
+            wpte = _packs(we, owner_e, kind_te, True)[1] if want_te else None
+            link_e = None
+            if grad_sum_e is not None and want_te:
+                grad_sum_e.total += 1
+                grad_sum_e.pending += 1
+                link_e = grad_sum_e
+            ctx.extra = (w_param_e, b_param_e, link_e, kind_te, Ke, be is not None, xe.shape)
+            y = _fwd_x3_seg([(x2, wp, b, lay == LAY_X), (xe2, wpe, be, False)], N, res2)
+        elif init_gather is not None:
             if kind != "x3" or res2 is not None:
                 raise ValueError("init_gather needs a layer on the bf16x3 kernel (gather_init_ok) without a residual")
             y = _fwd_x3_gather(x2, wp, N, b, init_gather, relu_in, relu_out)
@@ -978,19 +1067,31 @@
         ctx.has_bias, ctx.has_res = b is not None, residual is not None
         ctx.x_shape, ctx.k_orig, ctx.n_out, ctx.kind_t = x.shape, K, N, kind_t
         ctx.fwd_key = _param_key(w_param) if w_param is not None else None
-        ctx.save_for_backward(x2, wpt, y if (relu_out and not ctx.premasked and bits is None) else None, bits)
+        ctx.save_for_backward(x2, wpt, y if (relu_out and not ctx.premasked and bits is None) else None, bits, xe2, wpte)
         return y.reshape(*x.shape[:-1], N)
 
     @staticmethod
     def backward(ctx, dy):
         if dy is None:
-            return (None,) * 16
-        x2, wpt, y, bits = ctx.saved_tensors
+            return (None,) * 20
+        x2, wpt, y, bits, xe2, wpte = ctx.saved_tensors
         N = ctx.n_out
         dy2 = dy.reshape(-1, N)
         dy2 = dy2 if dy2.is_contiguous() else dy2.contiguous()
-        dx = dw = db = dres = None
+        dx = dw = db = dres = dxe = dwe = dbe = None
         lay = ctx.lay
+        if ctx.extra is not None:
+            w_param_e, b_param_e, link_e, kind_te, Ke, has_bias_e, xe_shape = ctx.extra
+            if w_param_e is not None:
+                if _use_side_stream(dy2):
+                    _wgrad_deferred(dy2, xe2, None, False, Ke, w_param_e, b_param_e)
+                else:
+                    wgrad_direct(dy2, xe2, None, False, Ke, w_param_e, b_param_e)
+            elif ctx.needs_input_grad[17] or (has_bias_e and ctx.needs_input_grad[18]):
+                dwe, dbe = _wgrad_sliced(dy2, xe2, None, False, has_bias_e, Ke)
+            if ctx.needs_input_grad[16]:
+                dxe = _plain_dx(link_e, kind_te, dy2, wpte, Ke)
+                dxe = dxe.reshape(xe_shape) if dxe is not None else None
         if ctx.w_param is not None:
             fn = None
             if lay:
@@ -1027,16 +1128,20 @@
                 addend, ctx.skip_dst.buf = ctx.skip_dst.buf, None
                 if addend is not None and addend.shape[1] != x2.shape[1]:
                     raise RuntimeError("SkipGrad: the skip gradient does not have the layer's input width")
-            dx = _run(ctx.kind_t, dyk, wpt, x2.shape[1], None, link.buf if link is not None else None, mk,
-                      x2 if (ctx.relu_in or ctx.mask_dx) else None, False, False, addend=addend,
-                      lay=(LAY_X if lay == LAY_Y else LAY_Y if lay == LAY_X else 0), mask_bits=bits)
-            dx = dx[:, :ctx.k_orig].reshape(ctx.x_shape) if ctx.k_orig != dx.shape[1] else dx.reshape(ctx.x_shape)
-            if link is not None:
-                link.pending -= 1
-                if link.pending > 0:
-                    link.buf, dx = dx.reshape(-1, ctx.k_orig), None
-                else:
-                    link.buf, link.pending = None, link.total
+            if mk is None and addend is None and not lay and bits is None and not (ctx.relu_in or ctx.mask_dx):
+                dx = _plain_dx(link, ctx.kind_t, dyk, wpt, x2.shape[1])
+            else:
+                dx = _run(ctx.kind_t, dyk, wpt, x2.shape[1], None, link.flush(x2.shape[1]) if link is not None else None, mk,
+                          x2 if (ctx.relu_in or ctx.mask_dx) else None, False, False, addend=addend,
+                          lay=(LAY_X if lay == LAY_Y else LAY_Y if lay == LAY_X else 0), mask_bits=bits)
+                if link is not None:
+                    link.pending -= 1
+                    if link.pending > 0:
+                        link.buf, dx = dx.reshape(-1, ctx.k_orig), None
+                    else:
+                        link.buf, link.pending = None, link.total
+            if dx is not None:
+                dx = dx[:, :ctx.k_orig].reshape(ctx.x_shape) if ctx.k_orig != dx.shape[1] else dx.reshape(ctx.x_shape)
         if ctx.skip_src is not None:
             ctx.skip_src.buf = dy2
         elif ctx.has_res and ctx.needs_input_grad[3]:
@@ -1044,7 +1149,7 @@
             dres = dres.reshape(dy.shape)
             if ctx.res_sign != 1.0:
                 dres = -dres
-        return dx, dw, db, dres, None, None, None, None, None, None, None, None, None, None, None, None
+        return dx, dw, db, dres, None, None, None, None, None, None, None, None, None, None, None, None, dxe, dwe, dbe, None
 
 
 _PARAM_GRADS_DIRECT = os.environ.get("NSDP_PARAM_GRADS", "direct") != "autograd"
@@ -1069,15 +1174,27 @@
 
 def linear(x, weight, bias=None, relu_in=False, relu_out=False, residual=None, params=False, grad_sum=None,
            out_f32=False, premasked=False, mask_dx=False, init_gather=None, residual_sign=1.0,
-           skip_src=None, skip_dst=None, tail_src=None, tail_dst=None, pack_owner=None, lay=0):
+           skip_src=None, skip_dst=None, tail_src=None, tail_dst=None, pack_owner=None, lay=0, then=None):
+    if then is not None:
+        xe, we, be, gse = then
+        if not (SEG_FWD and not precision.is_bf16() and seg_pair_ok(x, weight, xe, we, relu_in or relu_out or premasked or mask_dx
+                                                                    or init_gather is not None or residual_sign != 1.0
+                                                                    or tail_src is not None or tail_dst is not None
+                                                                    or skip_dst is not None, lay, bias is not None)):
+            y = linear(x, weight, bias, relu_in, relu_out, residual, params, grad_sum, out_f32, premasked, mask_dx, init_gather,
+                       residual_sign, skip_src, skip_dst, tail_src, tail_dst, pack_owner, lay)
+            return linear(xe, we, be, residual=y, params=params, grad_sum=gse)
     bw = (1 if premasked else 0) | (2 if mask_dx else 0)
-    w_param = b_param = None
-    if (params and _PARAM_GRADS_DIRECT and torch.is_grad_enabled() and weight.requires_grad and weight.is_leaf
-            and not _observed(weight)):
-        w_param = weight
-        b_param = bias if (bias is not None and bias.requires_grad and bias.is_leaf) else None
-        if bias is not None and (b_param is None or _observed(bias)):
-            w_param = b_param = None
+
+    def direct(weight, bias):
+        if (params and _PARAM_GRADS_DIRECT and torch.is_grad_enabled() and weight.requires_grad and weight.is_leaf
+                and not _observed(weight)):
+            b_param = bias if (bias is not None and bias.requires_grad and bias.is_leaf) else None
+            if bias is not None and (b_param is None or _observed(bias)):
+                return None, None
+            return weight, b_param
+        return None, None
+    w_param, b_param = direct(weight, bias)
     w2 = weight.squeeze(-1) if weight.dim() == 3 else weight
     owner = weight if (params and weight.is_leaf) else None
     if pack_owner is not None:
@@ -1110,9 +1227,15 @@
         raise ValueError("a layer is either end of a SkipGrad link")
     skip = (skip_src, True) if skip_src is not None else (skip_dst, False) if skip_dst is not None else None
     tail = (tail_src, True) if tail_src is not None else (tail_dst, False) if tail_dst is not None else None
+    seg = (None, None, None, None)
+    if then is not None:
+        xe, we, be, gse = then
+        wpe, bpe = direct(we, be)
+        seg = ((xe, we.detach(), None if be is None else be.detach()) if wpe is not None else (xe, we, be))
+        seg += ((wpe, bpe, gse, we if (params and we.is_leaf) else None),)
     if w_param is not None:
         return _LinearFn.apply(x, w2.detach(), None if bias is None else bias.detach(), residual, bool(relu_in),
                                bool(relu_out), w_param, b_param, grad_sum, None, bw, init_gather,
-                               float(residual_sign), skip, tail, int(lay))
+                               float(residual_sign), skip, tail, int(lay), *seg)
     return _LinearFn.apply(x, w2, bias, residual, bool(relu_in), bool(relu_out), None, None, grad_sum, owner, bw,
-                           init_gather, float(residual_sign), skip, None, int(lay))
+                           init_gather, float(residual_sign), skip, None, int(lay), *seg)
diff --git a/nsdp_amd/model/decoder/blocks.py b/nsdp_amd/model/decoder/blocks.py
--- a/nsdp_amd/model/decoder/blocks.py
+++ b/nsdp_amd/model/decoder/blocks.py
@@ -87,15 +87,15 @@
         self.shortcut = None if size_in == size_out else nn.Linear(size_in, size_out, bias=False)
         nn.init.zeros_(self.fc_1.weight)
 
-    def forward(self, x):
+    def forward(self, x, then=None):
         x_s = x if self.shortcut is None else ops.linear(x, self.shortcut)
         if precision.is_bf16():
             h = ops.linear(x, self.fc_0, relu_in=True)
-            return ops.linear(h, self.fc_1, relu_in=True, residual=x_s)
+            return ops.linear(h, self.fc_1, relu_in=True, residual=x_s, then=then)
         pair = ops.PAIR_MASK and torch.is_grad_enabled()
         skip = ops.skip_grad(x) if self.shortcut is None else None
         g16 = not pair and ops.g16_pair(x, self.fc_0, self.fc_1, relu_in0=True)
         h = ops.linear(x, self.fc_0, relu_in=True, relu=True, premasked=pair, skip_dst=skip,
                        lay=ops.hip_linear.LAY_Y if g16 else 0)
         return ops.linear(h, self.fc_1, residual=x_s, mask_dx=pair, skip_src=skip,
-                          lay=ops.hip_linear.LAY_X if g16 else 0)
+                          lay=ops.hip_linear.LAY_X if g16 else 0, then=then)
diff --git a/nsdp_amd/model/decoder/crosstransformer_decoder.py b/nsdp_amd/model/decoder/crosstransformer_decoder.py
--- a/nsdp_amd/model/decoder/crosstransformer_decoder.py
+++ b/nsdp_amd/model/decoder/crosstransformer_decoder.py
@@ -52,6 +52,11 @@
 
     def _trunk(self, lat):
         fan = hip_linear.InputGradSum() if (torch.is_grad_enabled() and lat.requires_grad) else None
+        if hip_linear.SEG_FWD and torch.is_grad_enabled() and not precision.is_bf16() and self.n_blocks > 0:
+            net = ops.linear(lat, self.init_enc, grad_sum=fan, then=(lat, self.fc_c[0], fan))
+            for i in range(self.n_blocks):
+                net = self.blocks[i](net, then=(lat, self.fc_c[i + 1], fan) if i + 1 < self.n_blocks else None)
+            return ops.linear(net, self.fc_out, relu_in=True, out_f32=True)
         net = ops.linear(lat, self.init_enc, grad_sum=fan)
         for i in range(self.n_blocks):
             net = ops.linear(lat, self.fc_c[i], residual=net, grad_sum=fan)
diff --git a/nsdp_amd/model/ops.py b/nsdp_amd/model/ops.py
--- a/nsdp_amd/model/ops.py
+++ b/nsdp_amd/model/ops.py
@@ -146,11 +146,13 @@
 def linear(x: torch.Tensor, lin, relu: bool = False, relu_in: bool = False, residual=None, grad_sum=None,
            out_f32: bool = False, premasked: bool = False, mask_dx: bool = False,
            init_gather=None, residual_sign: float = 1.0, skip_src=None, skip_dst=None, tail_src=None,
-           tail_dst=None, lay: int = 0) -> torch.Tensor:
+           tail_dst=None, lay: int = 0, then=None) -> torch.Tensor:
+    if then is not None:
+        then = (then[0], then[1].weight, then[1].bias, then[2])
     return hip_linear.linear(x, lin.weight, lin.bias, relu_in=relu_in, relu_out=relu, residual=residual,
                              params=True, grad_sum=grad_sum, out_f32=out_f32, premasked=premasked, mask_dx=mask_dx,
                              init_gather=init_gather, residual_sign=residual_sign,
-                             skip_src=skip_src, skip_dst=skip_dst, tail_src=tail_src, tail_dst=tail_dst, lay=lay)
+                             skip_src=skip_src, skip_dst=skip_dst, tail_src=tail_src, tail_dst=tail_dst, lay=lay, then=then)
 
 
 def g16_pair(x: torch.Tensor, lin0, lin1, relu_in0: bool = False) -> bool:
```
